# supranational/sppark

Measured on AMD Instinct MI355X. Metric: MSM points/sec (BLS12-381 G1, 2^26 points), higher is better.
Workload: dtype u32

## Files before the change

### sppark_amd/csrc/ff/montx_dev.hpp

```cpp
#pragma once
#include "mont_dev.hpp"

namespace sppark_amd {

SPPARK_DEVFN void macx(u64& acc, u32 a, u32 b)
{
#if defined(__HIP_DEVICE_COMPILE__)
    asm("v_mad_u64_u32 %0, vcc, %1, %2, %0" : "+v"(acc) : "v"(a), "v"(b) : "vcc");
#else
    acc += (u64)a * b;
#endif
}
SPPARK_DEVFN void macxs(u64& acc, u32 a, u32 b)
{
#if defined(__HIP_DEVICE_COMPILE__)
    asm("v_mad_u64_u32 %0, vcc, %1, %2, %0" : "+v"(acc) : "v"(a), "s"(b) : "vcc");
#else
    acc += (u64)a * b;
#endif
}
SPPARK_DEVFN void macx2(u64& acc0, u32 a0, u32 b0, u64& acc1, u32 a1, u32 b1)
{
#if defined(__HIP_DEVICE_COMPILE__)
    asm("v_mad_u64_u32 %0, vcc, %2, %3, %0\n\tv_mad_u64_u32 %1, vcc, %4, %5, %1"
        : "+v"(acc0), "+v"(acc1) : "v"(a0), "v"(b0), "v"(a1), "v"(b1) : "vcc");
#else
    acc0 += (u64)a0 * b0; acc1 += (u64)a1 * b1;
#endif
}
SPPARK_DEVFN void macxs2(u64& acc0, u32 a0, u64& acc1, u32 a1, u32 b)
{
#if defined(__HIP_DEVICE_COMPILE__)
    asm("v_mad_u64_u32 %0, vcc, %2, %4, %0\n\tv_mad_u64_u32 %1, vcc, %3, %4, %1"
        : "+v"(acc0), "+v"(acc1) : "v"(a0), "v"(a1), "s"(b) : "vcc");
#else
    acc0 += (u64)a0 * b; acc1 += (u64)a1 * b;
#endif
}

#if defined(SPPARK_HOST_EMULATION) && defined(SPPARK_TRACK_BOUNDS)
extern "C" void sppark_bound_violation(const char* what, double got, double limit);
#endif
template<class P, int LB> struct montx_dev {
    static constexpr int NW = P::N;
    static constexpr int HEAD = LB <= 28 ? 8 : 6;
    static constexpr int NL = (P::NBITS + HEAD + LB - 1) / LB;
    static constexpr int CAP = 1 << (32 - LB);
    static constexpr int FAT_L = 1 << (31 - LB);
    static constexpr bool TIGHT = LB > 28;
    static constexpr bool FAT_M_OK = (double)NL * (4294967296.0 * (double)(1ull << LB) + (double)(1ull << LB) * (double)(1ull << LB))
                                     + 68719476736.0 < 18446744073709551616.0;
    static constexpr int MA_A0 = TIGHT ? 3 : FAT_L, MA_A1 = TIGHT ? 3 : 6;
    static constexpr int SQR_L = TIGHT ? 2 : 4;
    static constexpr int N = NL;
    static constexpr u32 MASK = (1u << LB) - 1;
    static constexpr int RBITS = LB * NL;
    static_assert((double)NL * (double)(1ull << 31) * (double)(1ull << LB) + (double)NL * (double)(1ull << LB) * (double)(1ull << LB)
                  < 18446744073709551616.0, "a column (one fat operand) must fit the 64-bit accumulator");
    u32 l[NL];

#if defined(SPPARK_HOST_EMULATION) && defined(SPPARK_TRACK_BOUNDS)
# define SPPARK_BND(...) __VA_ARGS__
    double bv = -1.0, bl = -1.0;
    static double rho()
    {
        double p = 0.0;
        for (int i = NW - 1; i >= 0; i--) p = p * 4294967296.0 + (double)P::MOD[i];
        double r = 1.0;
        for (int i = 0; i < RBITS; i++) r *= 2.0;
        return r / p;
    }
    static constexpr double FAT_LEFT = (double)(1u << (31 - LB));
    static void bnd(bool ok, const char* what, double got, double lim) { if (!ok) sppark_bound_violation(what, got, lim); }
    void bnd_set(double v, double lm) { bv = v; bl = lm; }
    void bnd_known(const char* what) const { bnd(bv >= 0.0 && bl >= 0.0, what, bv, 0.0); }
#else
# define SPPARK_BND(...)
#endif

    SPPARK_DEVFN static constexpr u32 limb_of(const u32* w, int j)
    {
        const int bit = LB * j, wi = bit >> 5, sh = bit & 31;
        if (wi >= NW) return 0;
        u64 two = w[wi];
        if (wi + 1 < NW) two |= (u64)w[wi + 1] << 32;
        return (u32)(two >> sh) & MASK;
    }
    SPPARK_DEVFN static constexpr u32 mod_limb(int j) { return limb_of(P::MOD, j); }

    struct limbs_t { u32 l[NL]; };
    SPPARK_DEVFN static constexpr limbs_t make_pow2(int e)
    {
        u32 w[NW] = {};
        for (int i = 0; i < NW; i++) w[i] = P::ONE[i];
        for (int k = 0; k < e; k++) {
            u32 c = 0;
            for (int i = 0; i < NW; i++) { u32 t = (w[i] << 1) | c; c = w[i] >> 31; w[i] = t; }
            u32 d[NW] = {}; u64 bw = 0;
            for (int i = 0; i < NW; i++) { u64 t = (u64)w[i] - P::MOD[i] - bw; d[i] = (u32)t; bw = (t >> 63) & 1; }
            if (c || !bw) for (int i = 0; i < NW; i++) w[i] = d[i];
        }
        limbs_t r{};
        for (int j = 0; j < NL; j++) r.l[j] = limb_of(w, j);
        return r;
    }
    template<int E> struct pow2_tab { static constexpr limbs_t T = make_pow2(E); };
    SPPARK_DEVFN static constexpr limbs_t make_fat(int K, int B)
    {
        limbs_t r{}; u64 carry = 0;
        for (int j = 0; j < NL; j++) {
            u64 v = (u64)K * mod_limb(j) + carry; carry = v >> LB;
            r.l[j] = j == NL - 1 ? (u32)v : (u32)(v & MASK);
            if (j < NL - 1) r.l[j] += (u32)B << LB;
            if (j > 0) r.l[j] -= (u32)B;
        }
        return r;
    }
    template<int K, int B> struct fat_tab { static constexpr limbs_t T = make_fat(K, B); };
    template<int KMAX> struct multiples_t { u32 l[KMAX][NL]; };
    template<int KMAX> SPPARK_DEVFN static constexpr multiples_t<KMAX> make_multiples()
    {
        multiples_t<KMAX> r{};
        for (int k = 0; k < KMAX; k++) {
            u64 carry = 0;
            for (int j = 0; j < NL; j++) {
                u64 v = (u64)k * mod_limb(j) + carry; carry = v >> LB;
                r.l[k][j] = j == NL - 1 ? (u32)v : (u32)(v & MASK);
            }
        }
        return r;
    }
    template<int KMAX> struct multiples_tab { static constexpr multiples_t<KMAX> T = make_multiples<KMAX>(); };

    SPPARK_DEVFN static montx_dev one()
    {   montx_dev r; for (int j = 0; j < NL; j++) r.l[j] = pow2_tab<RBITS - 32 * NW>::T.l[j]; SPPARK_BND(r.bnd_set(1.0, 1.0);) return r;   }

    static constexpr int mod_bits()
    {
        int i = NW - 1;
        while (i > 0 && P::MOD[i] == 0) i--;
        int b = 32;
        while (b > 1 && !((P::MOD[i] >> (b - 1)) & 1)) b--;
        return 32 * i + b;
    }
    static constexpr int SH = RBITS - 32 * NW, PB = mod_bits(), TB = PB - 32;
    static_assert(SH >= 0 && SH < LB && SH <= 24 && PB > 64 && PB <= 32 * NW, "shift conversion: domain offset and modulus size");
    static constexpr u32 top32(const u32* w)
    {
        const int wi = TB >> 5, sh = TB & 31;
        u64 two = w[wi];
        if (wi + 1 < NW) two |= (u64)w[wi + 1] << 32;
        return (u32)(two >> sh);
    }
    static constexpr u64 PT = (u64)top32(P::MOD) + 1;
    static constexpr u32 QM = (u32)(((u64)1 << 62) / PT);
    SPPARK_DEVFN static constexpr u32 limb_of_shifted(const u32* w, int j)
    {
        const int bit = LB * j - SH;
        if (bit < 0) return (u32)((u64)w[0] << (-bit)) & MASK;
        const int wi = bit >> 5, sh = bit & 31;
        if (wi >= NW) return 0;
        u64 two = w[wi];
        if (wi + 1 < NW) two |= (u64)w[wi + 1] << 32;
        return j == NL - 1 ? (u32)(two >> sh) : (u32)(two >> sh) & MASK;
    }
    SPPARK_DEVFN static montx_dev from_std(const u32* w)
    {
        const u32 q = (u32)(((u64)top32(w) * QM) >> (62 - SH));
        montx_dev r;
        long long c = 0;
        #pragma unroll
        for (int j = 0; j < NL; j++) {
            c += (long long)limb_of_shifted(w, j) - (long long)((u64)q * mod_limb(j));
            r.l[j] = j == NL - 1 ? (u32)c : ((u32)c & MASK);
            c >>= LB;
        }
        SPPARK_BND(r.bnd_set(2.0, 1.0);)
        return r;
    }
    SPPARK_DEVFN void to_std(u32* w) const
    {
        montx_dev k;
        #pragma unroll
        for (int j = 0; j < NL; j++) k.l[j] = pow2_tab<0>::T.l[j];
        SPPARK_BND(k.bnd_set(1.0, 1.0);)
        (*this * k).cond_sub_p().to_words(w);
    }
    SPPARK_DEVFN montx_dev cond_sub_p() const
    {
        SPPARK_BND(bnd_known("cond_sub_p: operand"); bnd(bl <= 1.0, "cond_sub_p: normalised", bl, 1.0); bnd(bv <= 2.0, "cond_sub_p: < 2p", bv, 2.0);)
        montx_dev r = *this;
        SPPARK_BND(r.bnd_set(1.0, 1.0);)
        u32 d[NL]; int bw = 0;
        #pragma unroll
        for (int j = 0; j < NL; j++) {
            int v = (int)r.l[j] - (int)mod_limb(j) - bw;
            d[j] = j == NL - 1 ? (u32)v : ((u32)v & MASK); bw = (v >> 31) & 1;
        }
        #pragma unroll
        for (int j = 0; j < NL; j++) r.l[j] = bw ? r.l[j] : d[j];
        return r;
    }
    SPPARK_DEVFN static montx_dev from_words(const u32* w)
    {
        montx_dev a;
        #pragma unroll
        for (int j = 0; j < NL; j++) a.l[j] = limb_of(w, j);
        return a;
    }
    SPPARK_DEVFN void to_words(u32* w) const
    {
        #pragma unroll
        for (int i = 0; i < NW; i++) {
            const int bit = 32 * i, j = bit / LB, sh = bit % LB;
            u64 acc = (u64)l[j] >> sh;
            if (j + 1 < NL) acc |= (u64)l[j + 1] << (LB - sh);
            if (j + 2 < NL && 2 * LB - sh < 32) acc |= (u64)l[j + 2] << (2 * LB - sh);
            w[i] = (u32)acc;
        }
    }

    SPPARK_DEVFN static montx_dev from_wire(const u32* w)
    {   montx_dev r; for (int j = 0; j < NL; j++) r.l[j] = w[j]; return r;   }
    SPPARK_DEVFN void to_wire(u32* w) const { for (int j = 0; j < NL; j++) w[j] = l[j]; }

    SPPARK_DEVFN static montx_dev zero() { montx_dev r; for (int j = 0; j < NL; j++) r.l[j] = 0; SPPARK_BND(r.bnd_set(0.0, 0.0);) return r; }
    SPPARK_DEVFN bool limbs_all_zero() const
    {   u32 acc = l[0]; for (int j = 1; j < NL; j++) acc |= l[j]; return acc == 0;   }

    SPPARK_DEVFN montx_dev norm() const
    {
        montx_dev r; u32 c = 0;
        #pragma unroll
        for (int j = 0; j < NL - 1; j++) { u32 v = l[j] + c; r.l[j] = v & MASK; c = v >> LB; }
        r.l[NL - 1] = l[NL - 1] + c;
        SPPARK_BND(bnd_known("norm: operand"); bnd(bl <= (double)(CAP - 1), "norm: limbs", bl, (double)(CAP - 1)); r.bnd_set(bv, bl < 1.0 ? bl : 1.0);)
        return r;
    }

    SPPARK_DEVFN friend montx_dev operator+(const montx_dev& a, const montx_dev& b)
    {
        montx_dev r;
        #pragma unroll
        for (int j = 0; j < NL; j++) r.l[j] = a.l[j] + b.l[j];
        SPPARK_BND(a.bnd_known("+: left"); b.bnd_known("+: right"); r.bnd_set(a.bv + b.bv, a.bl + b.bl); bnd(r.bl < (double)CAP, "+: limbs wrap", r.bl, (double)CAP);)
        return r;
    }

    template<int K, int B = 1> SPPARK_DEVFN static montx_dev sub(const montx_dev& a, const montx_dev& b)
    {
        montx_dev r;
        #pragma unroll
        for (int j = 0; j < NL; j++) r.l[j] = a.l[j] + (fat_tab<K, B>::T.l[j] - b.l[j]);
        SPPARK_BND(a.bnd_known("sub: minuend"); b.bnd_known("sub: subtrahend");
                   bnd(b.bv <= (double)(K - 1), "sub<K>: subtrahend < (K-1) p", b.bv, (double)(K - 1));
                   bnd(b.bl <= (double)B, "sub<K,B>: subtrahend's limbs <= B 2^LB", b.bl, (double)B);
                   r.bnd_set(a.bv + (double)K, a.bl + (double)(B + 1));
                   bnd(r.bl < (double)CAP, "sub: limbs wrap", r.bl, (double)CAP);)
        return r;
    }
    template<int K, int B = 1> SPPARK_DEVFN static montx_dev neg(const montx_dev& b)
    {
        montx_dev r;
        #pragma unroll
        for (int j = 0; j < NL; j++) r.l[j] = fat_tab<K, B>::T.l[j] - b.l[j];
        SPPARK_BND(b.bnd_known("neg: operand");
                   bnd(b.bv <= (double)(K - 1), "neg<K>: operand < (K-1) p", b.bv, (double)(K - 1));
                   bnd(b.bl <= (double)B, "neg<K,B>: operand's limbs <= B 2^LB", b.bl, (double)B);
                   r.bnd_set((double)K, (double)(B + 1));)
        return r;
    }

    SPPARK_DEVFN static u64 shift_down(u64 A)
    {
#if defined(__HIP_DEVICE_COMPILE__)
        asm("v_lshrrev_b64 %0, %1, %0" : "+v"(A) : "n"(LB));
        return A;
#else
        return A >> LB;
#endif
    }

    SPPARK_DEVFN friend montx_dev operator*(const montx_dev& a, const montx_dev& b)
    {
        constexpr u32 PINV = P::M0 & MASK;
        u32 m[NL];
        montx_dev r;
        u64 A = 0;
        #pragma unroll
        for (int k = 0; k < 2 * NL; k++) {
            const int lo = k < NL ? 0 : k - NL + 1, hi = k < NL ? k : NL - 1;
            if (k <= 2 * NL - 2) {
                #pragma unroll
                for (int i = lo; i <= hi; i++) macx(A, a.l[i], b.l[k - i]);
                #pragma unroll
                for (int i = lo; i <= hi; i++) if (i < k) macxs(A, m[i], mod_limb(k - i));
            }
            if (k < NL) {
                m[k] = ((u32)A * PINV) & MASK;
                macxs(A, m[k], mod_limb(0));
            } else {
                r.l[k - NL] = (u32)A & MASK;
            }
            A = shift_down(A);
        }
        SPPARK_BND(a.bnd_known("*: left"); b.bnd_known("*: right");
                   bnd(b.bl <= 1.0, "*: right operand normalised", b.bl, 1.0);
                   bnd(a.bl <= FAT_LEFT + 1e-6, "*: left operand's limbs < 2^31", a.bl, FAT_LEFT);
                   r.bnd_set(a.bv * b.bv / rho() + 1.0, 1.0);)
        return r;
    }
    template<bool FAT_M> SPPARK_DEVFN static u32 quotient_digit(u64 A, int k)
    {
        constexpr u32 PINV = P::M0 & MASK;
        if (FAT_M && FAT_M_OK && k < NL - 1) return (u32)A * (u32)P::M0;
        return ((u32)A * PINV) & MASK;
    }

    template<bool NORM0 = false, bool NORM1 = false>
    SPPARK_DEVFN static void mul2(montx_dev& r0, montx_dev& r1,
                                  const montx_dev& a0, const montx_dev& b0,
                                  const montx_dev& a1, const montx_dev& b1)
    {
        u32 m0[NL], m1[NL];
        u64 A0 = 0, A1 = 0;
        #pragma unroll
        for (int k = 0; k < 2 * NL; k++) {
            const int lo = k < NL ? 0 : k - NL + 1, hi = k < NL ? k : NL - 1;
            if (k <= 2 * NL - 2) {
                #pragma unroll
                for (int i = lo; i <= hi; i++) macx2(A0, a0.l[i], b0.l[k - i], A1, a1.l[i], b1.l[k - i]);
                #pragma unroll
                for (int i = lo; i <= hi; i++) if (i < k) macxs2(A0, m0[i], A1, m1[i], mod_limb(k - i));
            }
            if (k < NL) {
                m0[k] = quotient_digit<NORM0>(A0, k); m1[k] = quotient_digit<NORM1>(A1, k);
                macxs2(A0, m0[k], A1, m1[k], mod_limb(0));
            } else {
                r0.l[k - NL] = (u32)A0 & MASK; r1.l[k - NL] = (u32)A1 & MASK;
            }
            A0 = shift_down(A0); A1 = shift_down(A1);
        }
        SPPARK_BND(a0.bnd_known("mul2: a0"); b0.bnd_known("mul2: b0"); a1.bnd_known("mul2: a1"); b1.bnd_known("mul2: b1");
                   bnd(b0.bl <= 1.0 && b1.bl <= 1.0, "mul2: right operands normalised", b0.bl > b1.bl ? b0.bl : b1.bl, 1.0);
                   bnd(a0.bl <= (NORM0 ? 1.0 : FAT_LEFT) + 1e-6, NORM0 ? "mul2<NORM0>: a0 normalised" : "mul2: a0's limbs < 2^31", a0.bl, NORM0 ? 1.0 : FAT_LEFT);
                   bnd(a1.bl <= (NORM1 ? 1.0 : FAT_LEFT) + 1e-6, NORM1 ? "mul2<NORM1>: a1 normalised" : "mul2: a1's limbs < 2^31", a1.bl, NORM1 ? 1.0 : FAT_LEFT);
                   r0.bnd_set(a0.bv * b0.bv / rho() + 1.0 + (NORM0 ? 1e-6 : 0.0), 1.0);
                   r1.bnd_set(a1.bv * b1.bv / rho() + 1.0 + (NORM1 ? 1e-6 : 0.0), 1.0);)
    }
    SPPARK_DEVFN static montx_dev mul_add(const montx_dev& a0, const montx_dev& b0,
                                          const montx_dev& a1, const montx_dev& b1)
    {
        static_assert((double)NL * ((double)MA_A0 + (double)MA_A1 + 1.0) * (double)(1ull << LB) * (double)(1ull << LB) + 68719476736.0
                      < 18446744073709551616.0, "a column of two products must fit the 64-bit accumulator");
        constexpr u32 PINV = P::M0 & MASK;
        u32 m[NL];
        montx_dev r;
        u64 A = 0;
        #pragma unroll
        for (int k = 0; k < 2 * NL; k++) {
            const int lo = k < NL ? 0 : k - NL + 1, hi = k < NL ? k : NL - 1;
            if (k <= 2 * NL - 2) {
                u64 B = 0;
                #pragma unroll
                for (int i = lo; i <= hi; i++) macx2(A, a0.l[i], b0.l[k - i], B, a1.l[i], b1.l[k - i]);
                const int mhi = hi < k ? hi : k - 1;
                #pragma unroll
                for (int i = lo; i + 1 <= mhi; i += 2) {
#if defined(__HIP_DEVICE_COMPILE__)
                    asm("v_mad_u64_u32 %0, vcc, %2, %4, %0\n\tv_mad_u64_u32 %1, vcc, %3, %5, %1"
                        : "+v"(A), "+v"(B) : "v"(m[i]), "v"(m[i + 1]), "s"(mod_limb(k - i)), "s"(mod_limb(k - i - 1)) : "vcc");
#else
                    A += (u64)m[i] * mod_limb(k - i); B += (u64)m[i + 1] * mod_limb(k - i - 1);
#endif
                }
                if (mhi >= lo && ((mhi - lo + 1) & 1)) macxs(A, m[mhi], mod_limb(k - mhi));
                A += B;
            }
            if (k < NL) {
                m[k] = ((u32)A * PINV) & MASK;
                macxs(A, m[k], mod_limb(0));
            } else {
                r.l[k - NL] = (u32)A & MASK;
            }
            A = shift_down(A);
        }
        SPPARK_BND(a0.bnd_known("mul_add: a0"); b0.bnd_known("mul_add: b0"); a1.bnd_known("mul_add: a1"); b1.bnd_known("mul_add: b1");
                   bnd(b0.bl <= 1.0 && b1.bl <= 1.0, "mul_add: right operands normalised", b0.bl > b1.bl ? b0.bl : b1.bl, 1.0);
                   bnd(a0.bl <= (double)MA_A0 + 1e-6, "mul_add: a0's limbs <= MA_A0 2^LB", a0.bl, (double)MA_A0);
                   bnd(a1.bl <= (double)MA_A1, "mul_add: a1's limbs <= MA_A1 2^LB", a1.bl, (double)MA_A1);
                   r.bnd_set((a0.bv * b0.bv + a1.bv * b1.bv) / rho() + 1.0, 1.0);)
        return r;
    }

    SPPARK_DEVFN static void sqr2(montx_dev& r0, montx_dev& r1, const montx_dev& a0, const montx_dev& a1)
    {
        u32 m0[NL], m1[NL], d0[NL], d1[NL];
        #pragma unroll
        for (int j = 0; j < NL; j++) { d0[j] = a0.l[j] << 1; d1[j] = a1.l[j] << 1; }
        u64 A0 = 0, A1 = 0;
        #pragma unroll
        for (int k = 0; k < 2 * NL; k++) {
            const int lo = k < NL ? 0 : k - NL + 1, hi = k < NL ? k : NL - 1;
            if (k <= 2 * NL - 2) {
                #pragma unroll
                for (int i = lo; i <= hi; i++) {
                    const int j = k - i;
                    if (i > j) continue;
                    if (i == j) macx2(A0, a0.l[i], a0.l[i], A1, a1.l[i], a1.l[i]);
                    else        macx2(A0, a0.l[i], d0[j], A1, a1.l[i], d1[j]);
                }
                #pragma unroll
                for (int i = lo; i <= hi; i++) if (i < k) macxs2(A0, m0[i], A1, m1[i], mod_limb(k - i));
            }
            if (k < NL) {
                m0[k] = quotient_digit<true>(A0, k); m1[k] = quotient_digit<true>(A1, k);
                macxs2(A0, m0[k], A1, m1[k], mod_limb(0));
            } else {
                r0.l[k - NL] = (u32)A0 & MASK; r1.l[k - NL] = (u32)A1 & MASK;
            }
            A0 = shift_down(A0); A1 = shift_down(A1);
        }
        SPPARK_BND(a0.bnd_known("sqr2: a0"); a1.bnd_known("sqr2: a1");
                   bnd(a0.bl <= 1.0 && a1.bl <= 1.0, "sqr2: operands normalised", a0.bl > a1.bl ? a0.bl : a1.bl, 1.0);
                   r0.bnd_set(a0.bv * a0.bv / rho() + 1.0 + 1e-6, 1.0); r1.bnd_set(a1.bv * a1.bv / rho() + 1.0 + 1e-6, 1.0);)
    }

    SPPARK_DEVFN montx_dev sqr() const
    {
        static_assert(((double)(NL / 2) * 2.0 * SQR_L * SQR_L + (double)(SQR_L * SQR_L) + (double)NL) * (double)(1ull << LB) * (double)(1ull << LB)
                      + 68719476736.0 < 18446744073709551616.0, "a column of a square of limbs <= SQR_L 2^LB must fit the 64-bit accumulator");
        constexpr u32 PINV = P::M0 & MASK;
        u32 m[NL], d[NL];
        #pragma unroll
        for (int j = 0; j < NL; j++) d[j] = l[j] << 1;
        montx_dev r;
        u64 A = 0;
        #pragma unroll
        for (int k = 0; k < 2 * NL; k++) {
            if (k <= 2 * NL - 2) {
                #pragma unroll
                for (int i = 0; i < NL; i++) {
                    const int j = k - i;
                    if (j < 0 || j >= NL || i > j) continue;
                    if (i == j) macx(A, l[i], l[i]);
                    else        macx(A, l[i], d[j]);
                }
                #pragma unroll
                for (int i = 0; i < NL; i++) {
                    const int j = k - i;
                    if (j < 0 || j >= NL || i >= k) continue;
                    macxs(A, m[i], mod_limb(j));
                }
            }
            if (k < NL) {
                m[k] = ((u32)A * PINV) & MASK;
                macxs(A, m[k], mod_limb(0));
            } else {
                r.l[k - NL] = (u32)A & MASK;
            }
            A = shift_down(A);
        }
        SPPARK_BND(bnd_known("sqr: operand"); bnd(bl <= (double)SQR_L, "sqr: limbs <= SQR_L 2^LB", bl, (double)SQR_L); r.bnd_set(bv * bv / rho() + 1.0, 1.0);)
        return r;
    }

    SPPARK_DEVFN montx_dev inverse() const
    {
        montx_dev r = one();
        bool started = false;
        #pragma unroll 1
        for (int w = NW - 1; w >= 0; w--) {
            u32 e = 0, borrow = 2;
            for (int k = 0; k <= w; k++) { e = P::MOD[k] - borrow; borrow = P::MOD[k] < borrow ? 1u : 0u; }
            #pragma unroll 1
            for (int b = 31; b >= 0; b--) {
                if (started) r = r.sqr();
                if ((e >> b) & 1u) { r = started ? r * *this : *this; started = true; }
            }
        }
        return r;
    }

    template<int KMAX> SPPARK_DEVFN bool is_zero_mod() const
    {
        SPPARK_BND(bnd_known("is_zero_mod: operand"); bnd(bl <= 1.0, "is_zero_mod: normalised", bl, 1.0);
                   bnd(bv <= (double)KMAX, "is_zero_mod<KMAX>: value < KMAX p", bv, (double)KMAX);)
        bool maybe = false;
        #pragma unroll
        for (int kk = 0; kk < KMAX; kk++) maybe |= (l[0] == multiples_tab<KMAX>::T.l[kk][0]);
        if (!maybe) return false;
        bool hit = false;
        #pragma unroll 1
        for (int k = 0; k < KMAX; k++) {
            u32 diff = 0;
            #pragma unroll
            for (int j = 0; j < NL; j++) diff |= multiples_tab<KMAX>::T.l[k][j] ^ l[j];
            hit |= diff == 0;
        }
        return hit;
    }
};

}
```

Before: 510.0 million.

## Emit each Montgomery product column as one fused inline-asm block

Replaces the per-term inline asm in the reduced-radix Montgomery multiply, square, mul2, sqr2 and mul_add loops with per-column asm blocks. Each block folds the previous quotient term, the shift, and all the column's a*b and m*p multiply-adds into a single asm statement, with modulus limbs passed as scalar operands. The aim is to remove compiler scheduling barriers and register copies between many tiny asm statements, giving a tight stream of v_mad_u64_u32 per column. It adds a large macro-generated header, and fixing the instruction order inside asm may block compiler interleaving or raise register pressure.

Result: faster. 519.7 million, median of 6 (+1.9%).

```diff
diff --git a/sppark_amd/csrc/ff/montx_blocks.hpp b/sppark_amd/csrc/ff/montx_blocks.hpp
--- /dev/null
+++ b/sppark_amd/csrc/ff/montx_blocks.hpp
@@ -0,0 +1,488 @@
+#pragma once
+namespace sppark_amd {
+#define MX_MAD(A, x, y) "v_mad_u64_u32 %[" #A "], vcc, %[" #x "], %[" #y "], %[" #A "]\n\t"
+#define MX_SHR(A)       "v_lshrrev_b64 %[" #A "], %[LB], %[" #A "]\n\t"
+#define MX_ADD(A, B)    "v_lshl_add_u64 %[" #A "], %[" #A "], 0, %[" #B "]\n\t"
+#define MX_V(name, e)   [name] "v"(e)
+#define MX_S(name, j)   [name] "s"(pl<F, j>)
+#define MX_ASM(text, outs, ...) asm(text : outs : __VA_ARGS__, [LB] "n"(F::LIMB_BITS) : "vcc")
+#define MX_ASM0(text, outs)     asm(text : outs : [LB] "n"(F::LIMB_BITS) : "vcc")
+#define MX_ACC1 [A] "+v"(A)
+#define MX_ACC2 [A0] "+v"(A0), [A1] "+v"(A1)
+#define MX_ACCS [A] "+v"(A), [B] "+v"(B)
+#define MX_I(j) (LO + j)
+#define MX_J(j) (K - LO - j)
+#define MX_MAX_TERMS 14
+#define MX_T_AB1_1 MX_MAD(A, x0_0, y0_0)
+#define MX_T_AB1_2 MX_T_AB1_1 MX_MAD(A, x0_1, y0_1)
+#define MX_T_AB1_3 MX_T_AB1_2 MX_MAD(A, x0_2, y0_2)
+#define MX_T_AB1_4 MX_T_AB1_3 MX_MAD(A, x0_3, y0_3)
+#define MX_T_AB1_5 MX_T_AB1_4 MX_MAD(A, x0_4, y0_4)
+#define MX_T_AB1_6 MX_T_AB1_5 MX_MAD(A, x0_5, y0_5)
+#define MX_T_AB1_7 MX_T_AB1_6 MX_MAD(A, x0_6, y0_6)
+#define MX_T_AB1_8 MX_T_AB1_7 MX_MAD(A, x0_7, y0_7)
+#define MX_T_AB1_9 MX_T_AB1_8 MX_MAD(A, x0_8, y0_8)
+#define MX_T_AB1_10 MX_T_AB1_9 MX_MAD(A, x0_9, y0_9)
+#define MX_T_AB1_11 MX_T_AB1_10 MX_MAD(A, x0_10, y0_10)
+#define MX_T_AB1_12 MX_T_AB1_11 MX_MAD(A, x0_11, y0_11)
+#define MX_T_AB1_13 MX_T_AB1_12 MX_MAD(A, x0_12, y0_12)
+#define MX_T_AB1_14 MX_T_AB1_13 MX_MAD(A, x0_13, y0_13)
+#define MX_O_AB1_1 MX_V(x0_0, o.x0(MX_I(0), MX_J(0))), MX_V(y0_0, o.y0(MX_I(0), MX_J(0)))
+#define MX_O_AB1_2 MX_O_AB1_1, MX_V(x0_1, o.x0(MX_I(1), MX_J(1))), MX_V(y0_1, o.y0(MX_I(1), MX_J(1)))
+#define MX_O_AB1_3 MX_O_AB1_2, MX_V(x0_2, o.x0(MX_I(2), MX_J(2))), MX_V(y0_2, o.y0(MX_I(2), MX_J(2)))
+#define MX_O_AB1_4 MX_O_AB1_3, MX_V(x0_3, o.x0(MX_I(3), MX_J(3))), MX_V(y0_3, o.y0(MX_I(3), MX_J(3)))
+#define MX_O_AB1_5 MX_O_AB1_4, MX_V(x0_4, o.x0(MX_I(4), MX_J(4))), MX_V(y0_4, o.y0(MX_I(4), MX_J(4)))
+#define MX_O_AB1_6 MX_O_AB1_5, MX_V(x0_5, o.x0(MX_I(5), MX_J(5))), MX_V(y0_5, o.y0(MX_I(5), MX_J(5)))
+#define MX_O_AB1_7 MX_O_AB1_6, MX_V(x0_6, o.x0(MX_I(6), MX_J(6))), MX_V(y0_6, o.y0(MX_I(6), MX_J(6)))
+#define MX_O_AB1_8 MX_O_AB1_7, MX_V(x0_7, o.x0(MX_I(7), MX_J(7))), MX_V(y0_7, o.y0(MX_I(7), MX_J(7)))
+#define MX_O_AB1_9 MX_O_AB1_8, MX_V(x0_8, o.x0(MX_I(8), MX_J(8))), MX_V(y0_8, o.y0(MX_I(8), MX_J(8)))
+#define MX_O_AB1_10 MX_O_AB1_9, MX_V(x0_9, o.x0(MX_I(9), MX_J(9))), MX_V(y0_9, o.y0(MX_I(9), MX_J(9)))
+#define MX_O_AB1_11 MX_O_AB1_10, MX_V(x0_10, o.x0(MX_I(10), MX_J(10))), MX_V(y0_10, o.y0(MX_I(10), MX_J(10)))
+#define MX_O_AB1_12 MX_O_AB1_11, MX_V(x0_11, o.x0(MX_I(11), MX_J(11))), MX_V(y0_11, o.y0(MX_I(11), MX_J(11)))
+#define MX_O_AB1_13 MX_O_AB1_12, MX_V(x0_12, o.x0(MX_I(12), MX_J(12))), MX_V(y0_12, o.y0(MX_I(12), MX_J(12)))
+#define MX_O_AB1_14 MX_O_AB1_13, MX_V(x0_13, o.x0(MX_I(13), MX_J(13))), MX_V(y0_13, o.y0(MX_I(13), MX_J(13)))
+#define MX_T_MP1_1 MX_MAD(A, m0_0, p_0)
+#define MX_T_MP1_2 MX_T_MP1_1 MX_MAD(A, m0_1, p_1)
+#define MX_T_MP1_3 MX_T_MP1_2 MX_MAD(A, m0_2, p_2)
+#define MX_T_MP1_4 MX_T_MP1_3 MX_MAD(A, m0_3, p_3)
+#define MX_T_MP1_5 MX_T_MP1_4 MX_MAD(A, m0_4, p_4)
+#define MX_T_MP1_6 MX_T_MP1_5 MX_MAD(A, m0_5, p_5)
+#define MX_T_MP1_7 MX_T_MP1_6 MX_MAD(A, m0_6, p_6)
+#define MX_T_MP1_8 MX_T_MP1_7 MX_MAD(A, m0_7, p_7)
+#define MX_T_MP1_9 MX_T_MP1_8 MX_MAD(A, m0_8, p_8)
+#define MX_T_MP1_10 MX_T_MP1_9 MX_MAD(A, m0_9, p_9)
+#define MX_T_MP1_11 MX_T_MP1_10 MX_MAD(A, m0_10, p_10)
+#define MX_T_MP1_12 MX_T_MP1_11 MX_MAD(A, m0_11, p_11)
+#define MX_T_MP1_13 MX_T_MP1_12 MX_MAD(A, m0_12, p_12)
+#define MX_T_MP1_14 MX_T_MP1_13 MX_MAD(A, m0_13, p_13)
+#define MX_O_MP1_1 MX_V(m0_0, o.m0(MX_I(0))), MX_S(p_0, MX_J(0))
+#define MX_O_MP1_2 MX_O_MP1_1, MX_V(m0_1, o.m0(MX_I(1))), MX_S(p_1, MX_J(1))
+#define MX_O_MP1_3 MX_O_MP1_2, MX_V(m0_2, o.m0(MX_I(2))), MX_S(p_2, MX_J(2))
+#define MX_O_MP1_4 MX_O_MP1_3, MX_V(m0_3, o.m0(MX_I(3))), MX_S(p_3, MX_J(3))
+#define MX_O_MP1_5 MX_O_MP1_4, MX_V(m0_4, o.m0(MX_I(4))), MX_S(p_4, MX_J(4))
+#define MX_O_MP1_6 MX_O_MP1_5, MX_V(m0_5, o.m0(MX_I(5))), MX_S(p_5, MX_J(5))
+#define MX_O_MP1_7 MX_O_MP1_6, MX_V(m0_6, o.m0(MX_I(6))), MX_S(p_6, MX_J(6))
+#define MX_O_MP1_8 MX_O_MP1_7, MX_V(m0_7, o.m0(MX_I(7))), MX_S(p_7, MX_J(7))
+#define MX_O_MP1_9 MX_O_MP1_8, MX_V(m0_8, o.m0(MX_I(8))), MX_S(p_8, MX_J(8))
+#define MX_O_MP1_10 MX_O_MP1_9, MX_V(m0_9, o.m0(MX_I(9))), MX_S(p_9, MX_J(9))
+#define MX_O_MP1_11 MX_O_MP1_10, MX_V(m0_10, o.m0(MX_I(10))), MX_S(p_10, MX_J(10))
+#define MX_O_MP1_12 MX_O_MP1_11, MX_V(m0_11, o.m0(MX_I(11))), MX_S(p_11, MX_J(11))
+#define MX_O_MP1_13 MX_O_MP1_12, MX_V(m0_12, o.m0(MX_I(12))), MX_S(p_12, MX_J(12))
+#define MX_O_MP1_14 MX_O_MP1_13, MX_V(m0_13, o.m0(MX_I(13))), MX_S(p_13, MX_J(13))
+#define MX_T_AB2_1(P, Q) MX_MAD(P, x0_0, y0_0) MX_MAD(Q, x1_0, y1_0)
+#define MX_T_AB2_2(P, Q) MX_T_AB2_1(P, Q) MX_MAD(P, x0_1, y0_1) MX_MAD(Q, x1_1, y1_1)
+#define MX_T_AB2_3(P, Q) MX_T_AB2_2(P, Q) MX_MAD(P, x0_2, y0_2) MX_MAD(Q, x1_2, y1_2)
+#define MX_T_AB2_4(P, Q) MX_T_AB2_3(P, Q) MX_MAD(P, x0_3, y0_3) MX_MAD(Q, x1_3, y1_3)
+#define MX_T_AB2_5(P, Q) MX_T_AB2_4(P, Q) MX_MAD(P, x0_4, y0_4) MX_MAD(Q, x1_4, y1_4)
+#define MX_T_AB2_6(P, Q) MX_T_AB2_5(P, Q) MX_MAD(P, x0_5, y0_5) MX_MAD(Q, x1_5, y1_5)
+#define MX_T_AB2_7(P, Q) MX_T_AB2_6(P, Q) MX_MAD(P, x0_6, y0_6) MX_MAD(Q, x1_6, y1_6)
+#define MX_T_AB2_8(P, Q) MX_T_AB2_7(P, Q) MX_MAD(P, x0_7, y0_7) MX_MAD(Q, x1_7, y1_7)
+#define MX_T_AB2_9(P, Q) MX_T_AB2_8(P, Q) MX_MAD(P, x0_8, y0_8) MX_MAD(Q, x1_8, y1_8)
+#define MX_T_AB2_10(P, Q) MX_T_AB2_9(P, Q) MX_MAD(P, x0_9, y0_9) MX_MAD(Q, x1_9, y1_9)
+#define MX_T_AB2_11(P, Q) MX_T_AB2_10(P, Q) MX_MAD(P, x0_10, y0_10) MX_MAD(Q, x1_10, y1_10)
+#define MX_T_AB2_12(P, Q) MX_T_AB2_11(P, Q) MX_MAD(P, x0_11, y0_11) MX_MAD(Q, x1_11, y1_11)
+#define MX_T_AB2_13(P, Q) MX_T_AB2_12(P, Q) MX_MAD(P, x0_12, y0_12) MX_MAD(Q, x1_12, y1_12)
+#define MX_T_AB2_14(P, Q) MX_T_AB2_13(P, Q) MX_MAD(P, x0_13, y0_13) MX_MAD(Q, x1_13, y1_13)
+#define MX_O_AB2_1 MX_V(x0_0, o.x0(MX_I(0), MX_J(0))), MX_V(y0_0, o.y0(MX_I(0), MX_J(0))), MX_V(x1_0, o.x1(MX_I(0), MX_J(0))), MX_V(y1_0, o.y1(MX_I(0), MX_J(0)))
+#define MX_O_AB2_2 MX_O_AB2_1, MX_V(x0_1, o.x0(MX_I(1), MX_J(1))), MX_V(y0_1, o.y0(MX_I(1), MX_J(1))), MX_V(x1_1, o.x1(MX_I(1), MX_J(1))), MX_V(y1_1, o.y1(MX_I(1), MX_J(1)))
+#define MX_O_AB2_3 MX_O_AB2_2, MX_V(x0_2, o.x0(MX_I(2), MX_J(2))), MX_V(y0_2, o.y0(MX_I(2), MX_J(2))), MX_V(x1_2, o.x1(MX_I(2), MX_J(2))), MX_V(y1_2, o.y1(MX_I(2), MX_J(2)))
+#define MX_O_AB2_4 MX_O_AB2_3, MX_V(x0_3, o.x0(MX_I(3), MX_J(3))), MX_V(y0_3, o.y0(MX_I(3), MX_J(3))), MX_V(x1_3, o.x1(MX_I(3), MX_J(3))), MX_V(y1_3, o.y1(MX_I(3), MX_J(3)))
+#define MX_O_AB2_5 MX_O_AB2_4, MX_V(x0_4, o.x0(MX_I(4), MX_J(4))), MX_V(y0_4, o.y0(MX_I(4), MX_J(4))), MX_V(x1_4, o.x1(MX_I(4), MX_J(4))), MX_V(y1_4, o.y1(MX_I(4), MX_J(4)))
+#define MX_O_AB2_6 MX_O_AB2_5, MX_V(x0_5, o.x0(MX_I(5), MX_J(5))), MX_V(y0_5, o.y0(MX_I(5), MX_J(5))), MX_V(x1_5, o.x1(MX_I(5), MX_J(5))), MX_V(y1_5, o.y1(MX_I(5), MX_J(5)))
+#define MX_O_AB2_7 MX_O_AB2_6, MX_V(x0_6, o.x0(MX_I(6), MX_J(6))), MX_V(y0_6, o.y0(MX_I(6), MX_J(6))), MX_V(x1_6, o.x1(MX_I(6), MX_J(6))), MX_V(y1_6, o.y1(MX_I(6), MX_J(6)))
+#define MX_O_AB2_8 MX_O_AB2_7, MX_V(x0_7, o.x0(MX_I(7), MX_J(7))), MX_V(y0_7, o.y0(MX_I(7), MX_J(7))), MX_V(x1_7, o.x1(MX_I(7), MX_J(7))), MX_V(y1_7, o.y1(MX_I(7), MX_J(7)))
+#define MX_O_AB2_9 MX_O_AB2_8, MX_V(x0_8, o.x0(MX_I(8), MX_J(8))), MX_V(y0_8, o.y0(MX_I(8), MX_J(8))), MX_V(x1_8, o.x1(MX_I(8), MX_J(8))), MX_V(y1_8, o.y1(MX_I(8), MX_J(8)))
+#define MX_O_AB2_10 MX_O_AB2_9, MX_V(x0_9, o.x0(MX_I(9), MX_J(9))), MX_V(y0_9, o.y0(MX_I(9), MX_J(9))), MX_V(x1_9, o.x1(MX_I(9), MX_J(9))), MX_V(y1_9, o.y1(MX_I(9), MX_J(9)))
+#define MX_O_AB2_11 MX_O_AB2_10, MX_V(x0_10, o.x0(MX_I(10), MX_J(10))), MX_V(y0_10, o.y0(MX_I(10), MX_J(10))), MX_V(x1_10, o.x1(MX_I(10), MX_J(10))), MX_V(y1_10, o.y1(MX_I(10), MX_J(10)))
+#define MX_O_AB2_12 MX_O_AB2_11, MX_V(x0_11, o.x0(MX_I(11), MX_J(11))), MX_V(y0_11, o.y0(MX_I(11), MX_J(11))), MX_V(x1_11, o.x1(MX_I(11), MX_J(11))), MX_V(y1_11, o.y1(MX_I(11), MX_J(11)))
+#define MX_O_AB2_13 MX_O_AB2_12, MX_V(x0_12, o.x0(MX_I(12), MX_J(12))), MX_V(y0_12, o.y0(MX_I(12), MX_J(12))), MX_V(x1_12, o.x1(MX_I(12), MX_J(12))), MX_V(y1_12, o.y1(MX_I(12), MX_J(12)))
+#define MX_O_AB2_14 MX_O_AB2_13, MX_V(x0_13, o.x0(MX_I(13), MX_J(13))), MX_V(y0_13, o.y0(MX_I(13), MX_J(13))), MX_V(x1_13, o.x1(MX_I(13), MX_J(13))), MX_V(y1_13, o.y1(MX_I(13), MX_J(13)))
+#define MX_T_MP2_1 MX_MAD(A0, m0_0, p_0) MX_MAD(A1, m1_0, p_0)
+#define MX_T_MP2_2 MX_T_MP2_1 MX_MAD(A0, m0_1, p_1) MX_MAD(A1, m1_1, p_1)
+#define MX_T_MP2_3 MX_T_MP2_2 MX_MAD(A0, m0_2, p_2) MX_MAD(A1, m1_2, p_2)
+#define MX_T_MP2_4 MX_T_MP2_3 MX_MAD(A0, m0_3, p_3) MX_MAD(A1, m1_3, p_3)
+#define MX_T_MP2_5 MX_T_MP2_4 MX_MAD(A0, m0_4, p_4) MX_MAD(A1, m1_4, p_4)
+#define MX_T_MP2_6 MX_T_MP2_5 MX_MAD(A0, m0_5, p_5) MX_MAD(A1, m1_5, p_5)
+#define MX_T_MP2_7 MX_T_MP2_6 MX_MAD(A0, m0_6, p_6) MX_MAD(A1, m1_6, p_6)
+#define MX_T_MP2_8 MX_T_MP2_7 MX_MAD(A0, m0_7, p_7) MX_MAD(A1, m1_7, p_7)
+#define MX_T_MP2_9 MX_T_MP2_8 MX_MAD(A0, m0_8, p_8) MX_MAD(A1, m1_8, p_8)
+#define MX_T_MP2_10 MX_T_MP2_9 MX_MAD(A0, m0_9, p_9) MX_MAD(A1, m1_9, p_9)
+#define MX_T_MP2_11 MX_T_MP2_10 MX_MAD(A0, m0_10, p_10) MX_MAD(A1, m1_10, p_10)
+#define MX_T_MP2_12 MX_T_MP2_11 MX_MAD(A0, m0_11, p_11) MX_MAD(A1, m1_11, p_11)
+#define MX_T_MP2_13 MX_T_MP2_12 MX_MAD(A0, m0_12, p_12) MX_MAD(A1, m1_12, p_12)
+#define MX_T_MP2_14 MX_T_MP2_13 MX_MAD(A0, m0_13, p_13) MX_MAD(A1, m1_13, p_13)
+#define MX_O_MP2_1 MX_V(m0_0, o.m0(MX_I(0))), MX_V(m1_0, o.m1(MX_I(0))), MX_S(p_0, MX_J(0))
+#define MX_O_MP2_2 MX_O_MP2_1, MX_V(m0_1, o.m0(MX_I(1))), MX_V(m1_1, o.m1(MX_I(1))), MX_S(p_1, MX_J(1))
+#define MX_O_MP2_3 MX_O_MP2_2, MX_V(m0_2, o.m0(MX_I(2))), MX_V(m1_2, o.m1(MX_I(2))), MX_S(p_2, MX_J(2))
+#define MX_O_MP2_4 MX_O_MP2_3, MX_V(m0_3, o.m0(MX_I(3))), MX_V(m1_3, o.m1(MX_I(3))), MX_S(p_3, MX_J(3))
+#define MX_O_MP2_5 MX_O_MP2_4, MX_V(m0_4, o.m0(MX_I(4))), MX_V(m1_4, o.m1(MX_I(4))), MX_S(p_4, MX_J(4))
+#define MX_O_MP2_6 MX_O_MP2_5, MX_V(m0_5, o.m0(MX_I(5))), MX_V(m1_5, o.m1(MX_I(5))), MX_S(p_5, MX_J(5))
+#define MX_O_MP2_7 MX_O_MP2_6, MX_V(m0_6, o.m0(MX_I(6))), MX_V(m1_6, o.m1(MX_I(6))), MX_S(p_6, MX_J(6))
+#define MX_O_MP2_8 MX_O_MP2_7, MX_V(m0_7, o.m0(MX_I(7))), MX_V(m1_7, o.m1(MX_I(7))), MX_S(p_7, MX_J(7))
+#define MX_O_MP2_9 MX_O_MP2_8, MX_V(m0_8, o.m0(MX_I(8))), MX_V(m1_8, o.m1(MX_I(8))), MX_S(p_8, MX_J(8))
+#define MX_O_MP2_10 MX_O_MP2_9, MX_V(m0_9, o.m0(MX_I(9))), MX_V(m1_9, o.m1(MX_I(9))), MX_S(p_9, MX_J(9))
+#define MX_O_MP2_11 MX_O_MP2_10, MX_V(m0_10, o.m0(MX_I(10))), MX_V(m1_10, o.m1(MX_I(10))), MX_S(p_10, MX_J(10))
+#define MX_O_MP2_12 MX_O_MP2_11, MX_V(m0_11, o.m0(MX_I(11))), MX_V(m1_11, o.m1(MX_I(11))), MX_S(p_11, MX_J(11))
+#define MX_O_MP2_13 MX_O_MP2_12, MX_V(m0_12, o.m0(MX_I(12))), MX_V(m1_12, o.m1(MX_I(12))), MX_S(p_12, MX_J(12))
+#define MX_O_MP2_14 MX_O_MP2_13, MX_V(m0_13, o.m0(MX_I(13))), MX_V(m1_13, o.m1(MX_I(13))), MX_S(p_13, MX_J(13))
+#define MX_T_MPS_1 MX_MAD(A, m0_0, p_0)
+#define MX_T_MPS_2 MX_T_MPS_1 MX_MAD(B, m0_1, p_1)
+#define MX_T_MPS_3 MX_T_MPS_2 MX_MAD(A, m0_2, p_2)
+#define MX_T_MPS_4 MX_T_MPS_3 MX_MAD(B, m0_3, p_3)
+#define MX_T_MPS_5 MX_T_MPS_4 MX_MAD(A, m0_4, p_4)
+#define MX_T_MPS_6 MX_T_MPS_5 MX_MAD(B, m0_5, p_5)
+#define MX_T_MPS_7 MX_T_MPS_6 MX_MAD(A, m0_6, p_6)
+#define MX_T_MPS_8 MX_T_MPS_7 MX_MAD(B, m0_7, p_7)
+#define MX_T_MPS_9 MX_T_MPS_8 MX_MAD(A, m0_8, p_8)
+#define MX_T_MPS_10 MX_T_MPS_9 MX_MAD(B, m0_9, p_9)
+#define MX_T_MPS_11 MX_T_MPS_10 MX_MAD(A, m0_10, p_10)
+#define MX_T_MPS_12 MX_T_MPS_11 MX_MAD(B, m0_11, p_11)
+#define MX_T_MPS_13 MX_T_MPS_12 MX_MAD(A, m0_12, p_12)
+#define MX_T_MPS_14 MX_T_MPS_13 MX_MAD(B, m0_13, p_13)
+struct montx_blocks {
+    template<class F, int J> static constexpr u32 pl = F::mod_limb(J);
+    struct mul_ops {
+        const u32 *a0, *b0, *a1, *b1, *q0, *q1;
+        static constexpr int terms(int lo, int hi, int) { return hi - lo + 1; }
+        SPPARK_DEVFN u32 x0(int i, int) const { return a0[i]; }
+        SPPARK_DEVFN u32 y0(int, int j) const { return b0[j]; }
+        SPPARK_DEVFN u32 x1(int i, int) const { return a1[i]; }
+        SPPARK_DEVFN u32 y1(int, int j) const { return b1[j]; }
+        SPPARK_DEVFN u32 m0(int i) const { return q0[i]; }
+        SPPARK_DEVFN u32 m1(int i) const { return q1[i]; }
+    };
+    struct sqr_ops {
+        const u32 *a0, *d0, *a1, *d1, *q0, *q1;
+        static constexpr int terms(int lo, int, int k) { return k / 2 - lo + 1; }
+        SPPARK_DEVFN u32 x0(int i, int) const { return a0[i]; }
+        SPPARK_DEVFN u32 y0(int i, int j) const { return i == j ? a0[j] : d0[j]; }
+        SPPARK_DEVFN u32 x1(int i, int) const { return a1[i]; }
+        SPPARK_DEVFN u32 y1(int i, int j) const { return i == j ? a1[j] : d1[j]; }
+        SPPARK_DEVFN u32 m0(int i) const { return q0[i]; }
+        SPPARK_DEVFN u32 m1(int i) const { return q1[i]; }
+    };
+#define MX_SHAPE \
+    constexpr int NL = F::NL, LO = K < NL ? 0 : K - NL + 1, HI = K < NL ? K : NL - 1; \
+    constexpr bool LAST = K == 2 * NL - 1, CLOSE = K >= 1 && K <= NL; \
+    constexpr int NAB = LAST ? 0 : OPS::terms(LO, HI, K), NMP = LAST ? 0 : (HI < K ? HI : K - 1) - LO + 1; \
+    static_assert(K >= 0 && K < 2 * NL && NAB <= MX_MAX_TERMS && NMP <= MX_MAX_TERMS, "column")
+    template<class F, int K, class OPS> SPPARK_DEVFN static void col1(u64& A, const OPS& o)
+    {
+        MX_SHAPE;
+#if defined(__HIP_DEVICE_COMPILE__)
+        if constexpr (LAST) MX_ASM0(MX_SHR(A), MX_ACC1);
+        else if constexpr (K == 0) { static_assert(NAB == 1 && NMP == 0, "shape"); asm(MX_T_AB1_1 : MX_ACC1 : MX_O_AB1_1 : "vcc"); }
+        else if constexpr (CLOSE && NAB == 1 && NMP == 1) MX_ASM(MX_MAD(A, mc0, pc) MX_SHR(A) MX_T_AB1_1 MX_T_MP1_1, MX_ACC1, MX_V(mc0, o.m0(K - 1)), MX_S(pc, 0), MX_O_AB1_1, MX_O_MP1_1);
+        else if constexpr (CLOSE && NAB == 2 && NMP == 1) MX_ASM(MX_MAD(A, mc0, pc) MX_SHR(A) MX_T_AB1_2 MX_T_MP1_1, MX_ACC1, MX_V(mc0, o.m0(K - 1)), MX_S(pc, 0), MX_O_AB1_2, MX_O_MP1_1);
+        else if constexpr (CLOSE && NAB == 2 && NMP == 2) MX_ASM(MX_MAD(A, mc0, pc) MX_SHR(A) MX_T_AB1_2 MX_T_MP1_2, MX_ACC1, MX_V(mc0, o.m0(K - 1)), MX_S(pc, 0), MX_O_AB1_2, MX_O_MP1_2);
+        else if constexpr (CLOSE && NAB == 2 && NMP == 3) MX_ASM(MX_MAD(A, mc0, pc) MX_SHR(A) MX_T_AB1_2 MX_T_MP1_3, MX_ACC1, MX_V(mc0, o.m0(K - 1)), MX_S(pc, 0), MX_O_AB1_2, MX_O_MP1_3);
+        else if constexpr (CLOSE && NAB == 3 && NMP == 2) MX_ASM(MX_MAD(A, mc0, pc) MX_SHR(A) MX_T_AB1_3 MX_T_MP1_2, MX_ACC1, MX_V(mc0, o.m0(K - 1)), MX_S(pc, 0), MX_O_AB1_3, MX_O_MP1_2);
+        else if constexpr (CLOSE && NAB == 3 && NMP == 4) MX_ASM(MX_MAD(A, mc0, pc) MX_SHR(A) MX_T_AB1_3 MX_T_MP1_4, MX_ACC1, MX_V(mc0, o.m0(K - 1)), MX_S(pc, 0), MX_O_AB1_3, MX_O_MP1_4);
+        else if constexpr (CLOSE && NAB == 3 && NMP == 5) MX_ASM(MX_MAD(A, mc0, pc) MX_SHR(A) MX_T_AB1_3 MX_T_MP1_5, MX_ACC1, MX_V(mc0, o.m0(K - 1)), MX_S(pc, 0), MX_O_AB1_3, MX_O_MP1_5);
+        else if constexpr (CLOSE && NAB == 4 && NMP == 3) MX_ASM(MX_MAD(A, mc0, pc) MX_SHR(A) MX_T_AB1_4 MX_T_MP1_3, MX_ACC1, MX_V(mc0, o.m0(K - 1)), MX_S(pc, 0), MX_O_AB1_4, MX_O_MP1_3);
+        else if constexpr (CLOSE && NAB == 4 && NMP == 6) MX_ASM(MX_MAD(A, mc0, pc) MX_SHR(A) MX_T_AB1_4 MX_T_MP1_6, MX_ACC1, MX_V(mc0, o.m0(K - 1)), MX_S(pc, 0), MX_O_AB1_4, MX_O_MP1_6);
+        else if constexpr (CLOSE && NAB == 4 && NMP == 7) MX_ASM(MX_MAD(A, mc0, pc) MX_SHR(A) MX_T_AB1_4 MX_T_MP1_7, MX_ACC1, MX_V(mc0, o.m0(K - 1)), MX_S(pc, 0), MX_O_AB1_4, MX_O_MP1_7);
+        else if constexpr (CLOSE && NAB == 4 && NMP == 8) MX_ASM(MX_MAD(A, mc0, pc) MX_SHR(A) MX_T_AB1_4 MX_T_MP1_8, MX_ACC1, MX_V(mc0, o.m0(K - 1)), MX_S(pc, 0), MX_O_AB1_4, MX_O_MP1_8);
+        else if constexpr (CLOSE && NAB == 5 && NMP == 4) MX_ASM(MX_MAD(A, mc0, pc) MX_SHR(A) MX_T_AB1_5 MX_T_MP1_4, MX_ACC1, MX_V(mc0, o.m0(K - 1)), MX_S(pc, 0), MX_O_AB1_5, MX_O_MP1_4);
+        else if constexpr (CLOSE && NAB == 5 && NMP == 8) MX_ASM(MX_MAD(A, mc0, pc) MX_SHR(A) MX_T_AB1_5 MX_T_MP1_8, MX_ACC1, MX_V(mc0, o.m0(K - 1)), MX_S(pc, 0), MX_O_AB1_5, MX_O_MP1_8);
+        else if constexpr (CLOSE && NAB == 5 && NMP == 9) MX_ASM(MX_MAD(A, mc0, pc) MX_SHR(A) MX_T_AB1_5 MX_T_MP1_9, MX_ACC1, MX_V(mc0, o.m0(K - 1)), MX_S(pc, 0), MX_O_AB1_5, MX_O_MP1_9);
+        else if constexpr (CLOSE && NAB == 6 && NMP == 5) MX_ASM(MX_MAD(A, mc0, pc) MX_SHR(A) MX_T_AB1_6 MX_T_MP1_5, MX_ACC1, MX_V(mc0, o.m0(K - 1)), MX_S(pc, 0), MX_O_AB1_6, MX_O_MP1_5);
+        else if constexpr (CLOSE && NAB == 6 && NMP == 10) MX_ASM(MX_MAD(A, mc0, pc) MX_SHR(A) MX_T_AB1_6 MX_T_MP1_10, MX_ACC1, MX_V(mc0, o.m0(K - 1)), MX_S(pc, 0), MX_O_AB1_6, MX_O_MP1_10);
+        else if constexpr (CLOSE && NAB == 6 && NMP == 11) MX_ASM(MX_MAD(A, mc0, pc) MX_SHR(A) MX_T_AB1_6 MX_T_MP1_11, MX_ACC1, MX_V(mc0, o.m0(K - 1)), MX_S(pc, 0), MX_O_AB1_6, MX_O_MP1_11);
+        else if constexpr (CLOSE && NAB == 7 && NMP == 6) MX_ASM(MX_MAD(A, mc0, pc) MX_SHR(A) MX_T_AB1_7 MX_T_MP1_6, MX_ACC1, MX_V(mc0, o.m0(K - 1)), MX_S(pc, 0), MX_O_AB1_7, MX_O_MP1_6);
+        else if constexpr (CLOSE && NAB == 7 && NMP == 12) MX_ASM(MX_MAD(A, mc0, pc) MX_SHR(A) MX_T_AB1_7 MX_T_MP1_12, MX_ACC1, MX_V(mc0, o.m0(K - 1)), MX_S(pc, 0), MX_O_AB1_7, MX_O_MP1_12);
+        else if constexpr (CLOSE && NAB == 7 && NMP == 13) MX_ASM(MX_MAD(A, mc0, pc) MX_SHR(A) MX_T_AB1_7 MX_T_MP1_13, MX_ACC1, MX_V(mc0, o.m0(K - 1)), MX_S(pc, 0), MX_O_AB1_7, MX_O_MP1_13);
+        else if constexpr (CLOSE && NAB == 8 && NMP == 7) MX_ASM(MX_MAD(A, mc0, pc) MX_SHR(A) MX_T_AB1_8 MX_T_MP1_7, MX_ACC1, MX_V(mc0, o.m0(K - 1)), MX_S(pc, 0), MX_O_AB1_8, MX_O_MP1_7);
+        else if constexpr (CLOSE && NAB == 8 && NMP == 8) MX_ASM(MX_MAD(A, mc0, pc) MX_SHR(A) MX_T_AB1_8 MX_T_MP1_8, MX_ACC1, MX_V(mc0, o.m0(K - 1)), MX_S(pc, 0), MX_O_AB1_8, MX_O_MP1_8);
+        else if constexpr (CLOSE && NAB == 9 && NMP == 8) MX_ASM(MX_MAD(A, mc0, pc) MX_SHR(A) MX_T_AB1_9 MX_T_MP1_8, MX_ACC1, MX_V(mc0, o.m0(K - 1)), MX_S(pc, 0), MX_O_AB1_9, MX_O_MP1_8);
+        else if constexpr (CLOSE && NAB == 9 && NMP == 9) MX_ASM(MX_MAD(A, mc0, pc) MX_SHR(A) MX_T_AB1_9 MX_T_MP1_9, MX_ACC1, MX_V(mc0, o.m0(K - 1)), MX_S(pc, 0), MX_O_AB1_9, MX_O_MP1_9);
+        else if constexpr (CLOSE && NAB == 10 && NMP == 9) MX_ASM(MX_MAD(A, mc0, pc) MX_SHR(A) MX_T_AB1_10 MX_T_MP1_9, MX_ACC1, MX_V(mc0, o.m0(K - 1)), MX_S(pc, 0), MX_O_AB1_10, MX_O_MP1_9);
+        else if constexpr (CLOSE && NAB == 11 && NMP == 10) MX_ASM(MX_MAD(A, mc0, pc) MX_SHR(A) MX_T_AB1_11 MX_T_MP1_10, MX_ACC1, MX_V(mc0, o.m0(K - 1)), MX_S(pc, 0), MX_O_AB1_11, MX_O_MP1_10);
+        else if constexpr (CLOSE && NAB == 12 && NMP == 11) MX_ASM(MX_MAD(A, mc0, pc) MX_SHR(A) MX_T_AB1_12 MX_T_MP1_11, MX_ACC1, MX_V(mc0, o.m0(K - 1)), MX_S(pc, 0), MX_O_AB1_12, MX_O_MP1_11);
+        else if constexpr (CLOSE && NAB == 13 && NMP == 12) MX_ASM(MX_MAD(A, mc0, pc) MX_SHR(A) MX_T_AB1_13 MX_T_MP1_12, MX_ACC1, MX_V(mc0, o.m0(K - 1)), MX_S(pc, 0), MX_O_AB1_13, MX_O_MP1_12);
+        else if constexpr (CLOSE && NAB == 13 && NMP == 13) MX_ASM(MX_MAD(A, mc0, pc) MX_SHR(A) MX_T_AB1_13 MX_T_MP1_13, MX_ACC1, MX_V(mc0, o.m0(K - 1)), MX_S(pc, 0), MX_O_AB1_13, MX_O_MP1_13);
+        else if constexpr (CLOSE && NAB == 14 && NMP == 13) MX_ASM(MX_MAD(A, mc0, pc) MX_SHR(A) MX_T_AB1_14 MX_T_MP1_13, MX_ACC1, MX_V(mc0, o.m0(K - 1)), MX_S(pc, 0), MX_O_AB1_14, MX_O_MP1_13);
+        else if constexpr (!CLOSE && NAB == 1 && NMP == 1) MX_ASM(MX_SHR(A) MX_T_AB1_1 MX_T_MP1_1, MX_ACC1, MX_O_AB1_1, MX_O_MP1_1);
+        else if constexpr (!CLOSE && NAB == 1 && NMP == 2) MX_ASM(MX_SHR(A) MX_T_AB1_1 MX_T_MP1_2, MX_ACC1, MX_O_AB1_1, MX_O_MP1_2);
+        else if constexpr (!CLOSE && NAB == 2 && NMP == 2) MX_ASM(MX_SHR(A) MX_T_AB1_2 MX_T_MP1_2, MX_ACC1, MX_O_AB1_2, MX_O_MP1_2);
+        else if constexpr (!CLOSE && NAB == 2 && NMP == 3) MX_ASM(MX_SHR(A) MX_T_AB1_2 MX_T_MP1_3, MX_ACC1, MX_O_AB1_2, MX_O_MP1_3);
+        else if constexpr (!CLOSE && NAB == 2 && NMP == 4) MX_ASM(MX_SHR(A) MX_T_AB1_2 MX_T_MP1_4, MX_ACC1, MX_O_AB1_2, MX_O_MP1_4);
+        else if constexpr (!CLOSE && NAB == 3 && NMP == 3) MX_ASM(MX_SHR(A) MX_T_AB1_3 MX_T_MP1_3, MX_ACC1, MX_O_AB1_3, MX_O_MP1_3);
+        else if constexpr (!CLOSE && NAB == 3 && NMP == 5) MX_ASM(MX_SHR(A) MX_T_AB1_3 MX_T_MP1_5, MX_ACC1, MX_O_AB1_3, MX_O_MP1_5);
+        else if constexpr (!CLOSE && NAB == 3 && NMP == 6) MX_ASM(MX_SHR(A) MX_T_AB1_3 MX_T_MP1_6, MX_ACC1, MX_O_AB1_3, MX_O_MP1_6);
+        else if constexpr (!CLOSE && NAB == 4 && NMP == 4) MX_ASM(MX_SHR(A) MX_T_AB1_4 MX_T_MP1_4, MX_ACC1, MX_O_AB1_4, MX_O_MP1_4);
+        else if constexpr (!CLOSE && NAB == 4 && NMP == 7) MX_ASM(MX_SHR(A) MX_T_AB1_4 MX_T_MP1_7, MX_ACC1, MX_O_AB1_4, MX_O_MP1_7);
+        else if constexpr (!CLOSE && NAB == 4 && NMP == 8) MX_ASM(MX_SHR(A) MX_T_AB1_4 MX_T_MP1_8, MX_ACC1, MX_O_AB1_4, MX_O_MP1_8);
+        else if constexpr (!CLOSE && NAB == 5 && NMP == 5) MX_ASM(MX_SHR(A) MX_T_AB1_5 MX_T_MP1_5, MX_ACC1, MX_O_AB1_5, MX_O_MP1_5);
+        else if constexpr (!CLOSE && NAB == 5 && NMP == 9) MX_ASM(MX_SHR(A) MX_T_AB1_5 MX_T_MP1_9, MX_ACC1, MX_O_AB1_5, MX_O_MP1_9);
+        else if constexpr (!CLOSE && NAB == 5 && NMP == 10) MX_ASM(MX_SHR(A) MX_T_AB1_5 MX_T_MP1_10, MX_ACC1, MX_O_AB1_5, MX_O_MP1_10);
+        else if constexpr (!CLOSE && NAB == 6 && NMP == 6) MX_ASM(MX_SHR(A) MX_T_AB1_6 MX_T_MP1_6, MX_ACC1, MX_O_AB1_6, MX_O_MP1_6);
+        else if constexpr (!CLOSE && NAB == 6 && NMP == 11) MX_ASM(MX_SHR(A) MX_T_AB1_6 MX_T_MP1_11, MX_ACC1, MX_O_AB1_6, MX_O_MP1_11);
+        else if constexpr (!CLOSE && NAB == 6 && NMP == 12) MX_ASM(MX_SHR(A) MX_T_AB1_6 MX_T_MP1_12, MX_ACC1, MX_O_AB1_6, MX_O_MP1_12);
+        else if constexpr (!CLOSE && NAB == 7 && NMP == 7) MX_ASM(MX_SHR(A) MX_T_AB1_7 MX_T_MP1_7, MX_ACC1, MX_O_AB1_7, MX_O_MP1_7);
+        else if constexpr (!CLOSE && NAB == 8 && NMP == 8) MX_ASM(MX_SHR(A) MX_T_AB1_8 MX_T_MP1_8, MX_ACC1, MX_O_AB1_8, MX_O_MP1_8);
+        else if constexpr (!CLOSE && NAB == 9 && NMP == 9) MX_ASM(MX_SHR(A) MX_T_AB1_9 MX_T_MP1_9, MX_ACC1, MX_O_AB1_9, MX_O_MP1_9);
+        else if constexpr (!CLOSE && NAB == 10 && NMP == 10) MX_ASM(MX_SHR(A) MX_T_AB1_10 MX_T_MP1_10, MX_ACC1, MX_O_AB1_10, MX_O_MP1_10);
+        else if constexpr (!CLOSE && NAB == 11 && NMP == 11) MX_ASM(MX_SHR(A) MX_T_AB1_11 MX_T_MP1_11, MX_ACC1, MX_O_AB1_11, MX_O_MP1_11);
+        else if constexpr (!CLOSE && NAB == 12 && NMP == 12) MX_ASM(MX_SHR(A) MX_T_AB1_12 MX_T_MP1_12, MX_ACC1, MX_O_AB1_12, MX_O_MP1_12);
+        else static_assert(K < 0, "no block of this shape");
+#else
+        if constexpr (CLOSE) A += (u64)o.m0(K - 1) * F::mod_limb(0);
+        if constexpr (K > 0) A >>= F::LIMB_BITS;
+        for (int j = 0; j < NAB; j++) A += (u64)o.x0(MX_I(j), MX_J(j)) * o.y0(MX_I(j), MX_J(j));
+        for (int j = 0; j < NMP; j++) A += (u64)o.m0(MX_I(j)) * F::mod_limb(MX_J(j));
+#endif
+    }
+    template<class F, int K, class OPS> SPPARK_DEVFN static void col2(u64& A0, u64& A1, const OPS& o)
+    {
+        MX_SHAPE;
+#if defined(__HIP_DEVICE_COMPILE__)
+        if constexpr (LAST) MX_ASM0(MX_SHR(A0) MX_SHR(A1), MX_ACC2);
+        else if constexpr (K == 0) { static_assert(NAB == 1 && NMP == 0, "shape"); asm(MX_T_AB2_1(A0, A1) : MX_ACC2 : MX_O_AB2_1 : "vcc"); }
+        else if constexpr (CLOSE && NAB == 1 && NMP == 1) MX_ASM(MX_MAD(A0, mc0, pc) MX_MAD(A1, mc1, pc) MX_SHR(A0) MX_SHR(A1) MX_T_AB2_1(A0, A1) MX_T_MP2_1, MX_ACC2, MX_V(mc0, o.m0(K - 1)), MX_S(pc, 0), MX_V(mc1, o.m1(K - 1)), MX_O_AB2_1, MX_O_MP2_1);
+        else if constexpr (CLOSE && NAB == 2 && NMP == 1) MX_ASM(MX_MAD(A0, mc0, pc) MX_MAD(A1, mc1, pc) MX_SHR(A0) MX_SHR(A1) MX_T_AB2_2(A0, A1) MX_T_MP2_1, MX_ACC2, MX_V(mc0, o.m0(K - 1)), MX_S(pc, 0), MX_V(mc1, o.m1(K - 1)), MX_O_AB2_2, MX_O_MP2_1);
+        else if constexpr (CLOSE && NAB == 2 && NMP == 2) MX_ASM(MX_MAD(A0, mc0, pc) MX_MAD(A1, mc1, pc) MX_SHR(A0) MX_SHR(A1) MX_T_AB2_2(A0, A1) MX_T_MP2_2, MX_ACC2, MX_V(mc0, o.m0(K - 1)), MX_S(pc, 0), MX_V(mc1, o.m1(K - 1)), MX_O_AB2_2, MX_O_MP2_2);
+        else if constexpr (CLOSE && NAB == 2 && NMP == 3) MX_ASM(MX_MAD(A0, mc0, pc) MX_MAD(A1, mc1, pc) MX_SHR(A0) MX_SHR(A1) MX_T_AB2_2(A0, A1) MX_T_MP2_3, MX_ACC2, MX_V(mc0, o.m0(K - 1)), MX_S(pc, 0), MX_V(mc1, o.m1(K - 1)), MX_O_AB2_2, MX_O_MP2_3);
+        else if constexpr (CLOSE && NAB == 3 && NMP == 2) MX_ASM(MX_MAD(A0, mc0, pc) MX_MAD(A1, mc1, pc) MX_SHR(A0) MX_SHR(A1) MX_T_AB2_3(A0, A1) MX_T_MP2_2, MX_ACC2, MX_V(mc0, o.m0(K - 1)), MX_S(pc, 0), MX_V(mc1, o.m1(K - 1)), MX_O_AB2_3, MX_O_MP2_2);
+        else if constexpr (CLOSE && NAB == 3 && NMP == 4) MX_ASM(MX_MAD(A0, mc0, pc) MX_MAD(A1, mc1, pc) MX_SHR(A0) MX_SHR(A1) MX_T_AB2_3(A0, A1) MX_T_MP2_4, MX_ACC2, MX_V(mc0, o.m0(K - 1)), MX_S(pc, 0), MX_V(mc1, o.m1(K - 1)), MX_O_AB2_3, MX_O_MP2_4);
+        else if constexpr (CLOSE && NAB == 3 && NMP == 5) MX_ASM(MX_MAD(A0, mc0, pc) MX_MAD(A1, mc1, pc) MX_SHR(A0) MX_SHR(A1) MX_T_AB2_3(A0, A1) MX_T_MP2_5, MX_ACC2, MX_V(mc0, o.m0(K - 1)), MX_S(pc, 0), MX_V(mc1, o.m1(K - 1)), MX_O_AB2_3, MX_O_MP2_5);
+        else if constexpr (CLOSE && NAB == 4 && NMP == 3) MX_ASM(MX_MAD(A0, mc0, pc) MX_MAD(A1, mc1, pc) MX_SHR(A0) MX_SHR(A1) MX_T_AB2_4(A0, A1) MX_T_MP2_3, MX_ACC2, MX_V(mc0, o.m0(K - 1)), MX_S(pc, 0), MX_V(mc1, o.m1(K - 1)), MX_O_AB2_4, MX_O_MP2_3);
+        else if constexpr (CLOSE && NAB == 4 && NMP == 6) MX_ASM(MX_MAD(A0, mc0, pc) MX_MAD(A1, mc1, pc) MX_SHR(A0) MX_SHR(A1) MX_T_AB2_4(A0, A1) MX_T_MP2_6, MX_ACC2, MX_V(mc0, o.m0(K - 1)), MX_S(pc, 0), MX_V(mc1, o.m1(K - 1)), MX_O_AB2_4, MX_O_MP2_6);
+        else if constexpr (CLOSE && NAB == 4 && NMP == 7) MX_ASM(MX_MAD(A0, mc0, pc) MX_MAD(A1, mc1, pc) MX_SHR(A0) MX_SHR(A1) MX_T_AB2_4(A0, A1) MX_T_MP2_7, MX_ACC2, MX_V(mc0, o.m0(K - 1)), MX_S(pc, 0), MX_V(mc1, o.m1(K - 1)), MX_O_AB2_4, MX_O_MP2_7);
+        else if constexpr (CLOSE && NAB == 4 && NMP == 8) MX_ASM(MX_MAD(A0, mc0, pc) MX_MAD(A1, mc1, pc) MX_SHR(A0) MX_SHR(A1) MX_T_AB2_4(A0, A1) MX_T_MP2_8, MX_ACC2, MX_V(mc0, o.m0(K - 1)), MX_S(pc, 0), MX_V(mc1, o.m1(K - 1)), MX_O_AB2_4, MX_O_MP2_8);
+        else if constexpr (CLOSE && NAB == 5 && NMP == 4) MX_ASM(MX_MAD(A0, mc0, pc) MX_MAD(A1, mc1, pc) MX_SHR(A0) MX_SHR(A1) MX_T_AB2_5(A0, A1) MX_T_MP2_4, MX_ACC2, MX_V(mc0, o.m0(K - 1)), MX_S(pc, 0), MX_V(mc1, o.m1(K - 1)), MX_O_AB2_5, MX_O_MP2_4);
+        else if constexpr (CLOSE && NAB == 5 && NMP == 8) MX_ASM(MX_MAD(A0, mc0, pc) MX_MAD(A1, mc1, pc) MX_SHR(A0) MX_SHR(A1) MX_T_AB2_5(A0, A1) MX_T_MP2_8, MX_ACC2, MX_V(mc0, o.m0(K - 1)), MX_S(pc, 0), MX_V(mc1, o.m1(K - 1)), MX_O_AB2_5, MX_O_MP2_8);
+        else if constexpr (CLOSE && NAB == 5 && NMP == 9) MX_ASM(MX_MAD(A0, mc0, pc) MX_MAD(A1, mc1, pc) MX_SHR(A0) MX_SHR(A1) MX_T_AB2_5(A0, A1) MX_T_MP2_9, MX_ACC2, MX_V(mc0, o.m0(K - 1)), MX_S(pc, 0), MX_V(mc1, o.m1(K - 1)), MX_O_AB2_5, MX_O_MP2_9);
+        else if constexpr (CLOSE && NAB == 6 && NMP == 5) MX_ASM(MX_MAD(A0, mc0, pc) MX_MAD(A1, mc1, pc) MX_SHR(A0) MX_SHR(A1) MX_T_AB2_6(A0, A1) MX_T_MP2_5, MX_ACC2, MX_V(mc0, o.m0(K - 1)), MX_S(pc, 0), MX_V(mc1, o.m1(K - 1)), MX_O_AB2_6, MX_O_MP2_5);
+        else if constexpr (CLOSE && NAB == 6 && NMP == 10) MX_ASM(MX_MAD(A0, mc0, pc) MX_MAD(A1, mc1, pc) MX_SHR(A0) MX_SHR(A1) MX_T_AB2_6(A0, A1) MX_T_MP2_10, MX_ACC2, MX_V(mc0, o.m0(K - 1)), MX_S(pc, 0), MX_V(mc1, o.m1(K - 1)), MX_O_AB2_6, MX_O_MP2_10);
+        else if constexpr (CLOSE && NAB == 6 && NMP == 11) MX_ASM(MX_MAD(A0, mc0, pc) MX_MAD(A1, mc1, pc) MX_SHR(A0) MX_SHR(A1) MX_T_AB2_6(A0, A1) MX_T_MP2_11, MX_ACC2, MX_V(mc0, o.m0(K - 1)), MX_S(pc, 0), MX_V(mc1, o.m1(K - 1)), MX_O_AB2_6, MX_O_MP2_11);
+        else if constexpr (CLOSE && NAB == 7 && NMP == 6) MX_ASM(MX_MAD(A0, mc0, pc) MX_MAD(A1, mc1, pc) MX_SHR(A0) MX_SHR(A1) MX_T_AB2_7(A0, A1) MX_T_MP2_6, MX_ACC2, MX_V(mc0, o.m0(K - 1)), MX_S(pc, 0), MX_V(mc1, o.m1(K - 1)), MX_O_AB2_7, MX_O_MP2_6);
+        else if constexpr (CLOSE && NAB == 7 && NMP == 12) MX_ASM(MX_MAD(A0, mc0, pc) MX_MAD(A1, mc1, pc) MX_SHR(A0) MX_SHR(A1) MX_T_AB2_7(A0, A1) MX_T_MP2_12, MX_ACC2, MX_V(mc0, o.m0(K - 1)), MX_S(pc, 0), MX_V(mc1, o.m1(K - 1)), MX_O_AB2_7, MX_O_MP2_12);
+        else if constexpr (CLOSE && NAB == 7 && NMP == 13) MX_ASM(MX_MAD(A0, mc0, pc) MX_MAD(A1, mc1, pc) MX_SHR(A0) MX_SHR(A1) MX_T_AB2_7(A0, A1) MX_T_MP2_13, MX_ACC2, MX_V(mc0, o.m0(K - 1)), MX_S(pc, 0), MX_V(mc1, o.m1(K - 1)), MX_O_AB2_7, MX_O_MP2_13);
+        else if constexpr (CLOSE && NAB == 8 && NMP == 7) MX_ASM(MX_MAD(A0, mc0, pc) MX_MAD(A1, mc1, pc) MX_SHR(A0) MX_SHR(A1) MX_T_AB2_8(A0, A1) MX_T_MP2_7, MX_ACC2, MX_V(mc0, o.m0(K - 1)), MX_S(pc, 0), MX_V(mc1, o.m1(K - 1)), MX_O_AB2_8, MX_O_MP2_7);
+        else if constexpr (CLOSE && NAB == 8 && NMP == 8) MX_ASM(MX_MAD(A0, mc0, pc) MX_MAD(A1, mc1, pc) MX_SHR(A0) MX_SHR(A1) MX_T_AB2_8(A0, A1) MX_T_MP2_8, MX_ACC2, MX_V(mc0, o.m0(K - 1)), MX_S(pc, 0), MX_V(mc1, o.m1(K - 1)), MX_O_AB2_8, MX_O_MP2_8);
+        else if constexpr (CLOSE && NAB == 9 && NMP == 8) MX_ASM(MX_MAD(A0, mc0, pc) MX_MAD(A1, mc1, pc) MX_SHR(A0) MX_SHR(A1) MX_T_AB2_9(A0, A1) MX_T_MP2_8, MX_ACC2, MX_V(mc0, o.m0(K - 1)), MX_S(pc, 0), MX_V(mc1, o.m1(K - 1)), MX_O_AB2_9, MX_O_MP2_8);
+        else if constexpr (CLOSE && NAB == 9 && NMP == 9) MX_ASM(MX_MAD(A0, mc0, pc) MX_MAD(A1, mc1, pc) MX_SHR(A0) MX_SHR(A1) MX_T_AB2_9(A0, A1) MX_T_MP2_9, MX_ACC2, MX_V(mc0, o.m0(K - 1)), MX_S(pc, 0), MX_V(mc1, o.m1(K - 1)), MX_O_AB2_9, MX_O_MP2_9);
+        else if constexpr (CLOSE && NAB == 10 && NMP == 9) MX_ASM(MX_MAD(A0, mc0, pc) MX_MAD(A1, mc1, pc) MX_SHR(A0) MX_SHR(A1) MX_T_AB2_10(A0, A1) MX_T_MP2_9, MX_ACC2, MX_V(mc0, o.m0(K - 1)), MX_S(pc, 0), MX_V(mc1, o.m1(K - 1)), MX_O_AB2_10, MX_O_MP2_9);
+        else if constexpr (CLOSE && NAB == 11 && NMP == 10) MX_ASM(MX_MAD(A0, mc0, pc) MX_MAD(A1, mc1, pc) MX_SHR(A0) MX_SHR(A1) MX_T_AB2_11(A0, A1) MX_T_MP2_10, MX_ACC2, MX_V(mc0, o.m0(K - 1)), MX_S(pc, 0), MX_V(mc1, o.m1(K - 1)), MX_O_AB2_11, MX_O_MP2_10);
+        else if constexpr (CLOSE && NAB == 12 && NMP == 11) MX_ASM(MX_MAD(A0, mc0, pc) MX_MAD(A1, mc1, pc) MX_SHR(A0) MX_SHR(A1) MX_T_AB2_12(A0, A1) MX_T_MP2_11, MX_ACC2, MX_V(mc0, o.m0(K - 1)), MX_S(pc, 0), MX_V(mc1, o.m1(K - 1)), MX_O_AB2_12, MX_O_MP2_11);
+        else if constexpr (CLOSE && NAB == 13 && NMP == 12) MX_ASM(MX_MAD(A0, mc0, pc) MX_MAD(A1, mc1, pc) MX_SHR(A0) MX_SHR(A1) MX_T_AB2_13(A0, A1) MX_T_MP2_12, MX_ACC2, MX_V(mc0, o.m0(K - 1)), MX_S(pc, 0), MX_V(mc1, o.m1(K - 1)), MX_O_AB2_13, MX_O_MP2_12);
+        else if constexpr (CLOSE && NAB == 13 && NMP == 13) MX_ASM(MX_MAD(A0, mc0, pc) MX_MAD(A1, mc1, pc) MX_SHR(A0) MX_SHR(A1) MX_T_AB2_13(A0, A1) MX_T_MP2_13, MX_ACC2, MX_V(mc0, o.m0(K - 1)), MX_S(pc, 0), MX_V(mc1, o.m1(K - 1)), MX_O_AB2_13, MX_O_MP2_13);
+        else if constexpr (CLOSE && NAB == 14 && NMP == 13) MX_ASM(MX_MAD(A0, mc0, pc) MX_MAD(A1, mc1, pc) MX_SHR(A0) MX_SHR(A1) MX_T_AB2_14(A0, A1) MX_T_MP2_13, MX_ACC2, MX_V(mc0, o.m0(K - 1)), MX_S(pc, 0), MX_V(mc1, o.m1(K - 1)), MX_O_AB2_14, MX_O_MP2_13);
+        else if constexpr (!CLOSE && NAB == 1 && NMP == 1) MX_ASM(MX_SHR(A0) MX_SHR(A1) MX_T_AB2_1(A0, A1) MX_T_MP2_1, MX_ACC2, MX_O_AB2_1, MX_O_MP2_1);
+        else if constexpr (!CLOSE && NAB == 1 && NMP == 2) MX_ASM(MX_SHR(A0) MX_SHR(A1) MX_T_AB2_1(A0, A1) MX_T_MP2_2, MX_ACC2, MX_O_AB2_1, MX_O_MP2_2);
+        else if constexpr (!CLOSE && NAB == 2 && NMP == 2) MX_ASM(MX_SHR(A0) MX_SHR(A1) MX_T_AB2_2(A0, A1) MX_T_MP2_2, MX_ACC2, MX_O_AB2_2, MX_O_MP2_2);
+        else if constexpr (!CLOSE && NAB == 2 && NMP == 3) MX_ASM(MX_SHR(A0) MX_SHR(A1) MX_T_AB2_2(A0, A1) MX_T_MP2_3, MX_ACC2, MX_O_AB2_2, MX_O_MP2_3);
+        else if constexpr (!CLOSE && NAB == 2 && NMP == 4) MX_ASM(MX_SHR(A0) MX_SHR(A1) MX_T_AB2_2(A0, A1) MX_T_MP2_4, MX_ACC2, MX_O_AB2_2, MX_O_MP2_4);
+        else if constexpr (!CLOSE && NAB == 3 && NMP == 3) MX_ASM(MX_SHR(A0) MX_SHR(A1) MX_T_AB2_3(A0, A1) MX_T_MP2_3, MX_ACC2, MX_O_AB2_3, MX_O_MP2_3);
+        else if constexpr (!CLOSE && NAB == 3 && NMP == 5) MX_ASM(MX_SHR(A0) MX_SHR(A1) MX_T_AB2_3(A0, A1) MX_T_MP2_5, MX_ACC2, MX_O_AB2_3, MX_O_MP2_5);
+        else if constexpr (!CLOSE && NAB == 3 && NMP == 6) MX_ASM(MX_SHR(A0) MX_SHR(A1) MX_T_AB2_3(A0, A1) MX_T_MP2_6, MX_ACC2, MX_O_AB2_3, MX_O_MP2_6);
+        else if constexpr (!CLOSE && NAB == 4 && NMP == 4) MX_ASM(MX_SHR(A0) MX_SHR(A1) MX_T_AB2_4(A0, A1) MX_T_MP2_4, MX_ACC2, MX_O_AB2_4, MX_O_MP2_4);
+        else if constexpr (!CLOSE && NAB == 4 && NMP == 7) MX_ASM(MX_SHR(A0) MX_SHR(A1) MX_T_AB2_4(A0, A1) MX_T_MP2_7, MX_ACC2, MX_O_AB2_4, MX_O_MP2_7);
+        else if constexpr (!CLOSE && NAB == 4 && NMP == 8) MX_ASM(MX_SHR(A0) MX_SHR(A1) MX_T_AB2_4(A0, A1) MX_T_MP2_8, MX_ACC2, MX_O_AB2_4, MX_O_MP2_8);
+        else if constexpr (!CLOSE && NAB == 5 && NMP == 5) MX_ASM(MX_SHR(A0) MX_SHR(A1) MX_T_AB2_5(A0, A1) MX_T_MP2_5, MX_ACC2, MX_O_AB2_5, MX_O_MP2_5);
+        else if constexpr (!CLOSE && NAB == 5 && NMP == 9) MX_ASM(MX_SHR(A0) MX_SHR(A1) MX_T_AB2_5(A0, A1) MX_T_MP2_9, MX_ACC2, MX_O_AB2_5, MX_O_MP2_9);
+        else if constexpr (!CLOSE && NAB == 5 && NMP == 10) MX_ASM(MX_SHR(A0) MX_SHR(A1) MX_T_AB2_5(A0, A1) MX_T_MP2_10, MX_ACC2, MX_O_AB2_5, MX_O_MP2_10);
+        else if constexpr (!CLOSE && NAB == 6 && NMP == 6) MX_ASM(MX_SHR(A0) MX_SHR(A1) MX_T_AB2_6(A0, A1) MX_T_MP2_6, MX_ACC2, MX_O_AB2_6, MX_O_MP2_6);
+        else if constexpr (!CLOSE && NAB == 6 && NMP == 11) MX_ASM(MX_SHR(A0) MX_SHR(A1) MX_T_AB2_6(A0, A1) MX_T_MP2_11, MX_ACC2, MX_O_AB2_6, MX_O_MP2_11);
+        else if constexpr (!CLOSE && NAB == 6 && NMP == 12) MX_ASM(MX_SHR(A0) MX_SHR(A1) MX_T_AB2_6(A0, A1) MX_T_MP2_12, MX_ACC2, MX_O_AB2_6, MX_O_MP2_12);
+        else if constexpr (!CLOSE && NAB == 7 && NMP == 7) MX_ASM(MX_SHR(A0) MX_SHR(A1) MX_T_AB2_7(A0, A1) MX_T_MP2_7, MX_ACC2, MX_O_AB2_7, MX_O_MP2_7);
+        else if constexpr (!CLOSE && NAB == 8 && NMP == 8) MX_ASM(MX_SHR(A0) MX_SHR(A1) MX_T_AB2_8(A0, A1) MX_T_MP2_8, MX_ACC2, MX_O_AB2_8, MX_O_MP2_8);
+        else if constexpr (!CLOSE && NAB == 9 && NMP == 9) MX_ASM(MX_SHR(A0) MX_SHR(A1) MX_T_AB2_9(A0, A1) MX_T_MP2_9, MX_ACC2, MX_O_AB2_9, MX_O_MP2_9);
+        else if constexpr (!CLOSE && NAB == 10 && NMP == 10) MX_ASM(MX_SHR(A0) MX_SHR(A1) MX_T_AB2_10(A0, A1) MX_T_MP2_10, MX_ACC2, MX_O_AB2_10, MX_O_MP2_10);
+        else if constexpr (!CLOSE && NAB == 11 && NMP == 11) MX_ASM(MX_SHR(A0) MX_SHR(A1) MX_T_AB2_11(A0, A1) MX_T_MP2_11, MX_ACC2, MX_O_AB2_11, MX_O_MP2_11);
+        else if constexpr (!CLOSE && NAB == 12 && NMP == 12) MX_ASM(MX_SHR(A0) MX_SHR(A1) MX_T_AB2_12(A0, A1) MX_T_MP2_12, MX_ACC2, MX_O_AB2_12, MX_O_MP2_12);
+        else static_assert(K < 0, "no block of this shape");
+#else
+        if constexpr (CLOSE) { A0 += (u64)o.m0(K - 1) * F::mod_limb(0); A1 += (u64)o.m1(K - 1) * F::mod_limb(0); }
+        if constexpr (K > 0) { A0 >>= F::LIMB_BITS; A1 >>= F::LIMB_BITS; }
+        for (int j = 0; j < NAB; j++) { A0 += (u64)o.x0(MX_I(j), MX_J(j)) * o.y0(MX_I(j), MX_J(j)); A1 += (u64)o.x1(MX_I(j), MX_J(j)) * o.y1(MX_I(j), MX_J(j)); }
+        for (int j = 0; j < NMP; j++) { A0 += (u64)o.m0(MX_I(j)) * F::mod_limb(MX_J(j)); A1 += (u64)o.m1(MX_I(j)) * F::mod_limb(MX_J(j)); }
+#endif
+    }
+    template<class F, int K, class OPS> SPPARK_DEVFN static void col_sum(u64& A, const OPS& o)
+    {
+        MX_SHAPE;
+        [[maybe_unused]] u64 B = 0;
+#if defined(__HIP_DEVICE_COMPILE__)
+        if constexpr (LAST) MX_ASM0(MX_SHR(A), MX_ACC1);
+        else if constexpr (K == 0) { static_assert(NAB == 1 && NMP == 0, "shape"); asm(MX_T_AB2_1(A, B) MX_ADD(A, B) : MX_ACCS : MX_O_AB2_1 : "vcc"); }
+        else if constexpr (CLOSE && NAB == 2 && NMP == 1) MX_ASM(MX_MAD(A, mc0, pc) MX_SHR(A) MX_T_AB2_2(A, B) MX_T_MPS_1 MX_ADD(A, B), MX_ACCS, MX_V(mc0, o.m0(K - 1)), MX_S(pc, 0), MX_O_AB2_2, MX_O_MP1_1);
+        else if constexpr (CLOSE && NAB == 3 && NMP == 2) MX_ASM(MX_MAD(A, mc0, pc) MX_SHR(A) MX_T_AB2_3(A, B) MX_T_MPS_2 MX_ADD(A, B), MX_ACCS, MX_V(mc0, o.m0(K - 1)), MX_S(pc, 0), MX_O_AB2_3, MX_O_MP1_2);
+        else if constexpr (CLOSE && NAB == 4 && NMP == 3) MX_ASM(MX_MAD(A, mc0, pc) MX_SHR(A) MX_T_AB2_4(A, B) MX_T_MPS_3 MX_ADD(A, B), MX_ACCS, MX_V(mc0, o.m0(K - 1)), MX_S(pc, 0), MX_O_AB2_4, MX_O_MP1_3);
+        else if constexpr (CLOSE && NAB == 5 && NMP == 4) MX_ASM(MX_MAD(A, mc0, pc) MX_SHR(A) MX_T_AB2_5(A, B) MX_T_MPS_4 MX_ADD(A, B), MX_ACCS, MX_V(mc0, o.m0(K - 1)), MX_S(pc, 0), MX_O_AB2_5, MX_O_MP1_4);
+        else if constexpr (CLOSE && NAB == 6 && NMP == 5) MX_ASM(MX_MAD(A, mc0, pc) MX_SHR(A) MX_T_AB2_6(A, B) MX_T_MPS_5 MX_ADD(A, B), MX_ACCS, MX_V(mc0, o.m0(K - 1)), MX_S(pc, 0), MX_O_AB2_6, MX_O_MP1_5);
+        else if constexpr (CLOSE && NAB == 7 && NMP == 6) MX_ASM(MX_MAD(A, mc0, pc) MX_SHR(A) MX_T_AB2_7(A, B) MX_T_MPS_6 MX_ADD(A, B), MX_ACCS, MX_V(mc0, o.m0(K - 1)), MX_S(pc, 0), MX_O_AB2_7, MX_O_MP1_6);
+        else if constexpr (CLOSE && NAB == 8 && NMP == 7) MX_ASM(MX_MAD(A, mc0, pc) MX_SHR(A) MX_T_AB2_8(A, B) MX_T_MPS_7 MX_ADD(A, B), MX_ACCS, MX_V(mc0, o.m0(K - 1)), MX_S(pc, 0), MX_O_AB2_8, MX_O_MP1_7);
+        else if constexpr (CLOSE && NAB == 8 && NMP == 8) MX_ASM(MX_MAD(A, mc0, pc) MX_SHR(A) MX_T_AB2_8(A, B) MX_T_MPS_8 MX_ADD(A, B), MX_ACCS, MX_V(mc0, o.m0(K - 1)), MX_S(pc, 0), MX_O_AB2_8, MX_O_MP1_8);
+        else if constexpr (CLOSE && NAB == 9 && NMP == 8) MX_ASM(MX_MAD(A, mc0, pc) MX_SHR(A) MX_T_AB2_9(A, B) MX_T_MPS_8 MX_ADD(A, B), MX_ACCS, MX_V(mc0, o.m0(K - 1)), MX_S(pc, 0), MX_O_AB2_9, MX_O_MP1_8);
+        else if constexpr (CLOSE && NAB == 9 && NMP == 9) MX_ASM(MX_MAD(A, mc0, pc) MX_SHR(A) MX_T_AB2_9(A, B) MX_T_MPS_9 MX_ADD(A, B), MX_ACCS, MX_V(mc0, o.m0(K - 1)), MX_S(pc, 0), MX_O_AB2_9, MX_O_MP1_9);
+        else if constexpr (CLOSE && NAB == 10 && NMP == 9) MX_ASM(MX_MAD(A, mc0, pc) MX_SHR(A) MX_T_AB2_10(A, B) MX_T_MPS_9 MX_ADD(A, B), MX_ACCS, MX_V(mc0, o.m0(K - 1)), MX_S(pc, 0), MX_O_AB2_10, MX_O_MP1_9);
+        else if constexpr (CLOSE && NAB == 11 && NMP == 10) MX_ASM(MX_MAD(A, mc0, pc) MX_SHR(A) MX_T_AB2_11(A, B) MX_T_MPS_10 MX_ADD(A, B), MX_ACCS, MX_V(mc0, o.m0(K - 1)), MX_S(pc, 0), MX_O_AB2_11, MX_O_MP1_10);
+        else if constexpr (CLOSE && NAB == 12 && NMP == 11) MX_ASM(MX_MAD(A, mc0, pc) MX_SHR(A) MX_T_AB2_12(A, B) MX_T_MPS_11 MX_ADD(A, B), MX_ACCS, MX_V(mc0, o.m0(K - 1)), MX_S(pc, 0), MX_O_AB2_12, MX_O_MP1_11);
+        else if constexpr (CLOSE && NAB == 13 && NMP == 12) MX_ASM(MX_MAD(A, mc0, pc) MX_SHR(A) MX_T_AB2_13(A, B) MX_T_MPS_12 MX_ADD(A, B), MX_ACCS, MX_V(mc0, o.m0(K - 1)), MX_S(pc, 0), MX_O_AB2_13, MX_O_MP1_12);
+        else if constexpr (CLOSE && NAB == 13 && NMP == 13) MX_ASM(MX_MAD(A, mc0, pc) MX_SHR(A) MX_T_AB2_13(A, B) MX_T_MPS_13 MX_ADD(A, B), MX_ACCS, MX_V(mc0, o.m0(K - 1)), MX_S(pc, 0), MX_O_AB2_13, MX_O_MP1_13);
+        else if constexpr (CLOSE && NAB == 14 && NMP == 13) MX_ASM(MX_MAD(A, mc0, pc) MX_SHR(A) MX_T_AB2_14(A, B) MX_T_MPS_13 MX_ADD(A, B), MX_ACCS, MX_V(mc0, o.m0(K - 1)), MX_S(pc, 0), MX_O_AB2_14, MX_O_MP1_13);
+        else if constexpr (!CLOSE && NAB == 1 && NMP == 1) MX_ASM(MX_SHR(A) MX_T_AB2_1(A, B) MX_T_MPS_1 MX_ADD(A, B), MX_ACCS, MX_O_AB2_1, MX_O_MP1_1);
+        else if constexpr (!CLOSE && NAB == 2 && NMP == 2) MX_ASM(MX_SHR(A) MX_T_AB2_2(A, B) MX_T_MPS_2 MX_ADD(A, B), MX_ACCS, MX_O_AB2_2, MX_O_MP1_2);
+        else if constexpr (!CLOSE && NAB == 3 && NMP == 3) MX_ASM(MX_SHR(A) MX_T_AB2_3(A, B) MX_T_MPS_3 MX_ADD(A, B), MX_ACCS, MX_O_AB2_3, MX_O_MP1_3);
+        else if constexpr (!CLOSE && NAB == 4 && NMP == 4) MX_ASM(MX_SHR(A) MX_T_AB2_4(A, B) MX_T_MPS_4 MX_ADD(A, B), MX_ACCS, MX_O_AB2_4, MX_O_MP1_4);
+        else if constexpr (!CLOSE && NAB == 5 && NMP == 5) MX_ASM(MX_SHR(A) MX_T_AB2_5(A, B) MX_T_MPS_5 MX_ADD(A, B), MX_ACCS, MX_O_AB2_5, MX_O_MP1_5);
+        else if constexpr (!CLOSE && NAB == 6 && NMP == 6) MX_ASM(MX_SHR(A) MX_T_AB2_6(A, B) MX_T_MPS_6 MX_ADD(A, B), MX_ACCS, MX_O_AB2_6, MX_O_MP1_6);
+        else if constexpr (!CLOSE && NAB == 7 && NMP == 7) MX_ASM(MX_SHR(A) MX_T_AB2_7(A, B) MX_T_MPS_7 MX_ADD(A, B), MX_ACCS, MX_O_AB2_7, MX_O_MP1_7);
+        else if constexpr (!CLOSE && NAB == 8 && NMP == 8) MX_ASM(MX_SHR(A) MX_T_AB2_8(A, B) MX_T_MPS_8 MX_ADD(A, B), MX_ACCS, MX_O_AB2_8, MX_O_MP1_8);
+        else if constexpr (!CLOSE && NAB == 9 && NMP == 9) MX_ASM(MX_SHR(A) MX_T_AB2_9(A, B) MX_T_MPS_9 MX_ADD(A, B), MX_ACCS, MX_O_AB2_9, MX_O_MP1_9);
+        else if constexpr (!CLOSE && NAB == 10 && NMP == 10) MX_ASM(MX_SHR(A) MX_T_AB2_10(A, B) MX_T_MPS_10 MX_ADD(A, B), MX_ACCS, MX_O_AB2_10, MX_O_MP1_10);
+        else if constexpr (!CLOSE && NAB == 11 && NMP == 11) MX_ASM(MX_SHR(A) MX_T_AB2_11(A, B) MX_T_MPS_11 MX_ADD(A, B), MX_ACCS, MX_O_AB2_11, MX_O_MP1_11);
+        else if constexpr (!CLOSE && NAB == 12 && NMP == 12) MX_ASM(MX_SHR(A) MX_T_AB2_12(A, B) MX_T_MPS_12 MX_ADD(A, B), MX_ACCS, MX_O_AB2_12, MX_O_MP1_12);
+        else static_assert(K < 0, "no block of this shape");
+#else
+        if constexpr (CLOSE) A += (u64)o.m0(K - 1) * F::mod_limb(0);
+        if constexpr (K > 0) A >>= F::LIMB_BITS;
+        for (int j = 0; j < NAB; j++) { A += (u64)o.x0(MX_I(j), MX_J(j)) * o.y0(MX_I(j), MX_J(j)); B += (u64)o.x1(MX_I(j), MX_J(j)) * o.y1(MX_I(j), MX_J(j)); }
+        for (int j = 0; j < NMP; j++) (j & 1 ? B : A) += (u64)o.m0(MX_I(j)) * F::mod_limb(MX_J(j));
+        A += B;
+#endif
+    }
+};
+#undef MX_MAD
+#undef MX_SHR
+#undef MX_ADD
+#undef MX_V
+#undef MX_S
+#undef MX_ASM
+#undef MX_ASM0
+#undef MX_ACC1
+#undef MX_ACC2
+#undef MX_ACCS
+#undef MX_I
+#undef MX_J
+#undef MX_SHAPE
+#undef MX_O_AB1_1
+#undef MX_O_AB1_10
+#undef MX_O_AB1_11
+#undef MX_O_AB1_12
+#undef MX_O_AB1_13
+#undef MX_O_AB1_14
+#undef MX_O_AB1_2
+#undef MX_O_AB1_3
+#undef MX_O_AB1_4
+#undef MX_O_AB1_5
+#undef MX_O_AB1_6
+#undef MX_O_AB1_7
+#undef MX_O_AB1_8
+#undef MX_O_AB1_9
+#undef MX_O_AB2_1
+#undef MX_O_AB2_10
+#undef MX_O_AB2_11
+#undef MX_O_AB2_12
+#undef MX_O_AB2_13
+#undef MX_O_AB2_14
+#undef MX_O_AB2_2
+#undef MX_O_AB2_3
+#undef MX_O_AB2_4
+#undef MX_O_AB2_5
+#undef MX_O_AB2_6
+#undef MX_O_AB2_7
+#undef MX_O_AB2_8
+#undef MX_O_AB2_9
+#undef MX_O_MP1_1
+#undef MX_O_MP1_10
+#undef MX_O_MP1_11
+#undef MX_O_MP1_12
+#undef MX_O_MP1_13
+#undef MX_O_MP1_14
+#undef MX_O_MP1_2
+#undef MX_O_MP1_3
+#undef MX_O_MP1_4
+#undef MX_O_MP1_5
+#undef MX_O_MP1_6
+#undef MX_O_MP1_7
+#undef MX_O_MP1_8
+#undef MX_O_MP1_9
+#undef MX_O_MP2_1
+#undef MX_O_MP2_10
+#undef MX_O_MP2_11
+#undef MX_O_MP2_12
+#undef MX_O_MP2_13
+#undef MX_O_MP2_14
+#undef MX_O_MP2_2
+#undef MX_O_MP2_3
+#undef MX_O_MP2_4
+#undef MX_O_MP2_5
+#undef MX_O_MP2_6
+#undef MX_O_MP2_7
+#undef MX_O_MP2_8
+#undef MX_O_MP2_9
+#undef MX_T_AB1_1
+#undef MX_T_AB1_10
+#undef MX_T_AB1_11
+#undef MX_T_AB1_12
+#undef MX_T_AB1_13
+#undef MX_T_AB1_14
+#undef MX_T_AB1_2
+#undef MX_T_AB1_3
+#undef MX_T_AB1_4
+#undef MX_T_AB1_5
+#undef MX_T_AB1_6
+#undef MX_T_AB1_7
+#undef MX_T_AB1_8
+#undef MX_T_AB1_9
+#undef MX_T_AB2_1
+#undef MX_T_AB2_10
+#undef MX_T_AB2_11
+#undef MX_T_AB2_12
+#undef MX_T_AB2_13
+#undef MX_T_AB2_14
+#undef MX_T_AB2_2
+#undef MX_T_AB2_3
+#undef MX_T_AB2_4
+#undef MX_T_AB2_5
+#undef MX_T_AB2_6
+#undef MX_T_AB2_7
+#undef MX_T_AB2_8
+#undef MX_T_AB2_9
+#undef MX_T_MP1_1
+#undef MX_T_MP1_10
+#undef MX_T_MP1_11
+#undef MX_T_MP1_12
+#undef MX_T_MP1_13
+#undef MX_T_MP1_14
+#undef MX_T_MP1_2
+#undef MX_T_MP1_3
+#undef MX_T_MP1_4
+#undef MX_T_MP1_5
+#undef MX_T_MP1_6
+#undef MX_T_MP1_7
+#undef MX_T_MP1_8
+#undef MX_T_MP1_9
+#undef MX_T_MP2_1
+#undef MX_T_MP2_10
+#undef MX_T_MP2_11
+#undef MX_T_MP2_12
+#undef MX_T_MP2_13
+#undef MX_T_MP2_14
+#undef MX_T_MP2_2
+#undef MX_T_MP2_3
+#undef MX_T_MP2_4
+#undef MX_T_MP2_5
+#undef MX_T_MP2_6
+#undef MX_T_MP2_7
+#undef MX_T_MP2_8
+#undef MX_T_MP2_9
+#undef MX_T_MPS_1
+#undef MX_T_MPS_10
+#undef MX_T_MPS_11
+#undef MX_T_MPS_12
+#undef MX_T_MPS_13
+#undef MX_T_MPS_14
+#undef MX_T_MPS_2
+#undef MX_T_MPS_3
+#undef MX_T_MPS_4
+#undef MX_T_MPS_5
+#undef MX_T_MPS_6
+#undef MX_T_MPS_7
+#undef MX_T_MPS_8
+#undef MX_T_MPS_9
+#undef MX_MAX_TERMS
+}
diff --git a/sppark_amd/csrc/ff/montx_dev.hpp b/sppark_amd/csrc/ff/montx_dev.hpp
--- a/sppark_amd/csrc/ff/montx_dev.hpp
+++ b/sppark_amd/csrc/ff/montx_dev.hpp
@@ -1,42 +1,10 @@
 #pragma once
 #include "mont_dev.hpp"
+#include "montx_blocks.hpp"
+#include <utility>
 
 namespace sppark_amd {
 
-SPPARK_DEVFN void macx(u64& acc, u32 a, u32 b)
-{
-#if defined(__HIP_DEVICE_COMPILE__)
-    asm("v_mad_u64_u32 %0, vcc, %1, %2, %0" : "+v"(acc) : "v"(a), "v"(b) : "vcc");
-#else
-    acc += (u64)a * b;
-#endif
-}
-SPPARK_DEVFN void macxs(u64& acc, u32 a, u32 b)
-{
-#if defined(__HIP_DEVICE_COMPILE__)
-    asm("v_mad_u64_u32 %0, vcc, %1, %2, %0" : "+v"(acc) : "v"(a), "s"(b) : "vcc");
-#else
-    acc += (u64)a * b;
-#endif
-}
-SPPARK_DEVFN void macx2(u64& acc0, u32 a0, u32 b0, u64& acc1, u32 a1, u32 b1)
-{
-#if defined(__HIP_DEVICE_COMPILE__)
-    asm("v_mad_u64_u32 %0, vcc, %2, %3, %0\n\tv_mad_u64_u32 %1, vcc, %4, %5, %1"
-        : "+v"(acc0), "+v"(acc1) : "v"(a0), "v"(b0), "v"(a1), "v"(b1) : "vcc");
-#else
-    acc0 += (u64)a0 * b0; acc1 += (u64)a1 * b1;
-#endif
-}
-SPPARK_DEVFN void macxs2(u64& acc0, u32 a0, u64& acc1, u32 a1, u32 b)
-{
-#if defined(__HIP_DEVICE_COMPILE__)
-    asm("v_mad_u64_u32 %0, vcc, %2, %4, %0\n\tv_mad_u64_u32 %1, vcc, %3, %4, %1"
-        : "+v"(acc0), "+v"(acc1) : "v"(a0), "v"(a1), "s"(b) : "vcc");
-#else
-    acc0 += (u64)a0 * b; acc1 += (u64)a1 * b;
-#endif
-}
 
 #if defined(SPPARK_HOST_EMULATION) && defined(SPPARK_TRACK_BOUNDS)
 extern "C" void sppark_bound_violation(const char* what, double got, double limit);
@@ -53,6 +21,12 @@
     static constexpr int MA_A0 = TIGHT ? 3 : FAT_L, MA_A1 = TIGHT ? 3 : 6;
     static constexpr int SQR_L = TIGHT ? 2 : 4;
     static constexpr int N = NL;
+    static constexpr int LIMB_BITS = LB;
+    typedef montx_blocks blk;
+    template<int K> struct col { static constexpr int value = K; };
+    template<class Fn, int... K> SPPARK_DEVFN static void for_columns(Fn& f, std::integer_sequence<int, K...>) { (f(col<K>()), ...); }
+    template<class Fn> SPPARK_DEVFN static void for_columns(Fn f) { for_columns(f, std::make_integer_sequence<int, 2 * NL>()); }
+# define SPPARK_COLUMN(kc, k) (auto kc) __attribute__((always_inline)) { constexpr int k = decltype(kc)::value;
     static constexpr u32 MASK = (1u << LB) - 1;
     static constexpr int RBITS = LB * NL;
     static_assert((double)NL * (double)(1ull << 31) * (double)(1ull << LB) + (double)NL * (double)(1ull << LB) * (double)(1ull << LB)
@@ -271,15 +245,6 @@
         return r;
     }
 
-    SPPARK_DEVFN static u64 shift_down(u64 A)
-    {
-#if defined(__HIP_DEVICE_COMPILE__)
-        asm("v_lshrrev_b64 %0, %1, %0" : "+v"(A) : "n"(LB));
-        return A;
-#else
-        return A >> LB;
-#endif
-    }
 
     SPPARK_DEVFN friend montx_dev operator*(const montx_dev& a, const montx_dev& b)
     {
@@ -287,23 +252,11 @@
         u32 m[NL];
         montx_dev r;
         u64 A = 0;
-        #pragma unroll
-        for (int k = 0; k < 2 * NL; k++) {
-            const int lo = k < NL ? 0 : k - NL + 1, hi = k < NL ? k : NL - 1;
-            if (k <= 2 * NL - 2) {
-                #pragma unroll
-                for (int i = lo; i <= hi; i++) macx(A, a.l[i], b.l[k - i]);
-                #pragma unroll
-                for (int i = lo; i <= hi; i++) if (i < k) macxs(A, m[i], mod_limb(k - i));
-            }
-            if (k < NL) {
-                m[k] = ((u32)A * PINV) & MASK;
-                macxs(A, m[k], mod_limb(0));
-            } else {
-                r.l[k - NL] = (u32)A & MASK;
-            }
-            A = shift_down(A);
-        }
+        for_columns([&] SPPARK_COLUMN(kc, k)
+            blk::template col1<montx_dev, k>(A, blk::mul_ops{a.l, b.l, nullptr, nullptr, m, nullptr});
+            if constexpr (k < NL) m[k] = ((u32)A * PINV) & MASK;
+            else        r.l[k - NL] = (u32)A & MASK;
+        });
         SPPARK_BND(a.bnd_known("*: left"); b.bnd_known("*: right");
                    bnd(b.bl <= 1.0, "*: right operand normalised", b.bl, 1.0);
                    bnd(a.bl <= FAT_LEFT + 1e-6, "*: left operand's limbs < 2^31", a.bl, FAT_LEFT);
@@ -324,23 +277,11 @@
     {
         u32 m0[NL], m1[NL];
         u64 A0 = 0, A1 = 0;
-        #pragma unroll
-        for (int k = 0; k < 2 * NL; k++) {
-            const int lo = k < NL ? 0 : k - NL + 1, hi = k < NL ? k : NL - 1;
-            if (k <= 2 * NL - 2) {
-                #pragma unroll
-                for (int i = lo; i <= hi; i++) macx2(A0, a0.l[i], b0.l[k - i], A1, a1.l[i], b1.l[k - i]);
-                #pragma unroll
-                for (int i = lo; i <= hi; i++) if (i < k) macxs2(A0, m0[i], A1, m1[i], mod_limb(k - i));
-            }
-            if (k < NL) {
-                m0[k] = quotient_digit<NORM0>(A0, k); m1[k] = quotient_digit<NORM1>(A1, k);
-                macxs2(A0, m0[k], A1, m1[k], mod_limb(0));
-            } else {
-                r0.l[k - NL] = (u32)A0 & MASK; r1.l[k - NL] = (u32)A1 & MASK;
-            }
-            A0 = shift_down(A0); A1 = shift_down(A1);
-        }
+        for_columns([&] SPPARK_COLUMN(kc, k)
+            blk::template col2<montx_dev, k>(A0, A1, blk::mul_ops{a0.l, b0.l, a1.l, b1.l, m0, m1});
+            if constexpr (k < NL) { m0[k] = quotient_digit<NORM0>(A0, k); m1[k] = quotient_digit<NORM1>(A1, k); }
+            else        { r0.l[k - NL] = (u32)A0 & MASK; r1.l[k - NL] = (u32)A1 & MASK; }
+        });
         SPPARK_BND(a0.bnd_known("mul2: a0"); b0.bnd_known("mul2: b0"); a1.bnd_known("mul2: a1"); b1.bnd_known("mul2: b1");
                    bnd(b0.bl <= 1.0 && b1.bl <= 1.0, "mul2: right operands normalised", b0.bl > b1.bl ? b0.bl : b1.bl, 1.0);
                    bnd(a0.bl <= (NORM0 ? 1.0 : FAT_LEFT) + 1e-6, NORM0 ? "mul2<NORM0>: a0 normalised" : "mul2: a0's limbs < 2^31", a0.bl, NORM0 ? 1.0 : FAT_LEFT);
@@ -357,34 +298,11 @@
         u32 m[NL];
         montx_dev r;
         u64 A = 0;
-        #pragma unroll
-        for (int k = 0; k < 2 * NL; k++) {
-            const int lo = k < NL ? 0 : k - NL + 1, hi = k < NL ? k : NL - 1;
-            if (k <= 2 * NL - 2) {
-                u64 B = 0;
-                #pragma unroll
-                for (int i = lo; i <= hi; i++) macx2(A, a0.l[i], b0.l[k - i], B, a1.l[i], b1.l[k - i]);
-                const int mhi = hi < k ? hi : k - 1;
-                #pragma unroll
-                for (int i = lo; i + 1 <= mhi; i += 2) {
-#if defined(__HIP_DEVICE_COMPILE__)
-                    asm("v_mad_u64_u32 %0, vcc, %2, %4, %0\n\tv_mad_u64_u32 %1, vcc, %3, %5, %1"
-                        : "+v"(A), "+v"(B) : "v"(m[i]), "v"(m[i + 1]), "s"(mod_limb(k - i)), "s"(mod_limb(k - i - 1)) : "vcc");
-#else
-                    A += (u64)m[i] * mod_limb(k - i); B += (u64)m[i + 1] * mod_limb(k - i - 1);
-#endif
-                }
-                if (mhi >= lo && ((mhi - lo + 1) & 1)) macxs(A, m[mhi], mod_limb(k - mhi));
-                A += B;
-            }
-            if (k < NL) {
-                m[k] = ((u32)A * PINV) & MASK;
-                macxs(A, m[k], mod_limb(0));
-            } else {
-                r.l[k - NL] = (u32)A & MASK;
-            }
-            A = shift_down(A);
-        }
+        for_columns([&] SPPARK_COLUMN(kc, k)
+            blk::template col_sum<montx_dev, k>(A, blk::mul_ops{a0.l, b0.l, a1.l, b1.l, m, nullptr});
+            if constexpr (k < NL) m[k] = ((u32)A * PINV) & MASK;
+            else        r.l[k - NL] = (u32)A & MASK;
+        });
         SPPARK_BND(a0.bnd_known("mul_add: a0"); b0.bnd_known("mul_add: b0"); a1.bnd_known("mul_add: a1"); b1.bnd_known("mul_add: b1");
                    bnd(b0.bl <= 1.0 && b1.bl <= 1.0, "mul_add: right operands normalised", b0.bl > b1.bl ? b0.bl : b1.bl, 1.0);
                    bnd(a0.bl <= (double)MA_A0 + 1e-6, "mul_add: a0's limbs <= MA_A0 2^LB", a0.bl, (double)MA_A0);
@@ -399,28 +317,11 @@
         #pragma unroll
         for (int j = 0; j < NL; j++) { d0[j] = a0.l[j] << 1; d1[j] = a1.l[j] << 1; }
         u64 A0 = 0, A1 = 0;
-        #pragma unroll
-        for (int k = 0; k < 2 * NL; k++) {
-            const int lo = k < NL ? 0 : k - NL + 1, hi = k < NL ? k : NL - 1;
-            if (k <= 2 * NL - 2) {
-                #pragma unroll
-                for (int i = lo; i <= hi; i++) {
-                    const int j = k - i;
-                    if (i > j) continue;
-                    if (i == j) macx2(A0, a0.l[i], a0.l[i], A1, a1.l[i], a1.l[i]);
-                    else        macx2(A0, a0.l[i], d0[j], A1, a1.l[i], d1[j]);
-                }
-                #pragma unroll
-                for (int i = lo; i <= hi; i++) if (i < k) macxs2(A0, m0[i], A1, m1[i], mod_limb(k - i));
-            }
-            if (k < NL) {
-                m0[k] = quotient_digit<true>(A0, k); m1[k] = quotient_digit<true>(A1, k);
-                macxs2(A0, m0[k], A1, m1[k], mod_limb(0));
-            } else {
-                r0.l[k - NL] = (u32)A0 & MASK; r1.l[k - NL] = (u32)A1 & MASK;
-            }
-            A0 = shift_down(A0); A1 = shift_down(A1);
-        }
+        for_columns([&] SPPARK_COLUMN(kc, k)
+            blk::template col2<montx_dev, k>(A0, A1, blk::sqr_ops{a0.l, d0, a1.l, d1, m0, m1});
+            if constexpr (k < NL) { m0[k] = quotient_digit<true>(A0, k); m1[k] = quotient_digit<true>(A1, k); }
+            else        { r0.l[k - NL] = (u32)A0 & MASK; r1.l[k - NL] = (u32)A1 & MASK; }
+        });
         SPPARK_BND(a0.bnd_known("sqr2: a0"); a1.bnd_known("sqr2: a1");
                    bnd(a0.bl <= 1.0 && a1.bl <= 1.0, "sqr2: operands normalised", a0.bl > a1.bl ? a0.bl : a1.bl, 1.0);
                    r0.bnd_set(a0.bv * a0.bv / rho() + 1.0 + 1e-6, 1.0); r1.bnd_set(a1.bv * a1.bv / rho() + 1.0 + 1e-6, 1.0);)
@@ -436,31 +337,11 @@
         for (int j = 0; j < NL; j++) d[j] = l[j] << 1;
         montx_dev r;
         u64 A = 0;
-        #pragma unroll
-        for (int k = 0; k < 2 * NL; k++) {
-            if (k <= 2 * NL - 2) {
-                #pragma unroll
-                for (int i = 0; i < NL; i++) {
-                    const int j = k - i;
-                    if (j < 0 || j >= NL || i > j) continue;
-                    if (i == j) macx(A, l[i], l[i]);
-                    else        macx(A, l[i], d[j]);
-                }
-                #pragma unroll
-                for (int i = 0; i < NL; i++) {
-                    const int j = k - i;
-                    if (j < 0 || j >= NL || i >= k) continue;
-                    macxs(A, m[i], mod_limb(j));
-                }
-            }
-            if (k < NL) {
-                m[k] = ((u32)A * PINV) & MASK;
-                macxs(A, m[k], mod_limb(0));
-            } else {
-                r.l[k - NL] = (u32)A & MASK;
-            }
-            A = shift_down(A);
-        }
+        for_columns([&] SPPARK_COLUMN(kc, k)
+            blk::template col1<montx_dev, k>(A, blk::sqr_ops{l, d, nullptr, nullptr, m, nullptr});
+            if constexpr (k < NL) m[k] = ((u32)A * PINV) & MASK;
+            else        r.l[k - NL] = (u32)A & MASK;
+        });
         SPPARK_BND(bnd_known("sqr: operand"); bnd(bl <= (double)SQR_L, "sqr: limbs <= SQR_L 2^LB", bl, (double)SQR_L); r.bnd_set(bv * bv / rho() + 1.0, 1.0);)
         return r;
     }
```
